# JuanJoZP/cfd-hemodynamic

Measured on NVIDIA B200. Metric: DOF-timesteps/s, higher is better.
Workload: dtype f64

## Files before the change

### cfd_hemodynamic_b200/_lib.py

```python
from __future__ import annotations

import ctypes as C
import os

import numpy as np

_HERE = os.path.dirname(os.path.abspath(__file__))
LIB_PATH = os.path.join(_HERE, "libhemo_sm100.so")

HEMO_DIVERGED = -100
Q_FU, Q_FP, Q_UU, Q_UP, Q_PU, Q_PP = range(6)
CELL_TRIANGLE, CELL_QUADRILATERAL, CELL_TETRAHEDRON, CELL_TRIANGLE_P2 = 0, 1, 2, 3


class HemoError(RuntimeError):
    pass


class HemoDiverged(HemoError):
    pass


class Params(C.Structure):
    _fields_ = [("dt", C.c_double), ("rho", C.c_double), ("mu", C.c_double),
# ... 53 lines not shown
    "hemo_remove_mean_vec": (_I, [_VP, _L, _VP]),
    "hemo_amg_set_level": (_I, [_VP, _I, _I, _I, _I] + [_VP] * 10),
    "hemo_amg_finalize": (_I, [_VP, _I, _I]),
    "hemo_host_aggregate": (_I, [_I, _VP, _VP, _VP, _VP, C.POINTER(_I)]),
    "hemo_set_solver_opts": (_I, [_VP, C.POINTER(SolverOpts)]),
    "hemo_set_pc_mask": (_I, [_VP, _VP]),
    "hemo_set_external_schur": (_I, [_VP, _I]),
    "hemo_amg_setup_scalar": (_I, [_VP, _VP, _D]),
    "hemo_mask_nodes": (_I, [_VP, _VP, _VP]),
    "hemo_vec_mdot": (_I, [_VP, _L, _I, _VP, _L, _VP, _VP]),
    "hemo_vec_maxpy": (_I, [_VP, _L, _I, _VP, _L, _VP, _D, _VP, C.POINTER(_D)]),
    "hemo_vec_scale": (_I, [_VP, _L, _D, _VP, _VP]),
    "hemo_use_graph": (_I, [_VP, _I]),
    "hemo_set_schur_mask": (_I, [_VP, _VP]),
    "hemo_pc_set_schur_operator": (_I, [_VP, _VP, _VP, _VP, _D, _D]),
    "hemo_amg_set_fine_pattern": (_I, [_VP, _I, _VP, _VP]),
    "hemo_pc_set_schur_selfp": (_I, [_VP, _VP, _D]),
    "hemo_pc_set_convection": (_I, [_VP, _VP, _VP, _D]),
    "hemo_pc_setup": (_I, [_VP, _VP, _VP, _VP]),
    "hemo_amg_apply": (_I, [_VP, _I, _VP, _VP, _I]),
    "hemo_amg_get_level_values": (_I, [_VP, _I, _I, _VP, _L]),
    "hemo_pc_apply": (_I, [_VP, _VP, _VP, _VP]),
    "hemo_fgmres": (_I, [_VP, _VP, _VP, _VP, C.POINTER(_I), C.POINTER(_D)]),
    "hemo_comm_unique_id": (_I, [C.c_char_p]),
    "hemo_comm_init": (_I, [_VP, C.c_char_p, _I, _I]),
    "hemo_comm_info": (_I, [_VP, C.POINTER(_I), C.POINTER(_I), C.POINTER(_I), C.POINTER(_L), C.POINTER(_L)]),
    "hemo_comm_set_partition": (_I, [_VP, _I, _I, _VP, _VP, _VP, _VP, _I]),
    "hemo_set_graph": (_I, [_VP, _I, _VP, _VP, _L]),
    "hemo_pc_set_coarse_pressure": (_I, [_VP, _VP, _I] + [_VP] * 6 + [_I]),
    "hemo_comm_halo_update": (_I, [_VP, _VP]),
    "hemo_comm_allreduce": (_I, [_VP, _VP, _I]),
    "hemo_global_dot": (_I, [_VP, _VP, _VP, C.POINTER(_D)]),
    "hemo_set_poll_interval": (_I, [_VP, _I]),
}

_lib = None


def load_library(path: str | None = None):
    global _lib
    if _lib is not None and path is None:
        return _lib
    p = path or LIB_PATH
    if not os.path.exists(p):
        raise HemoError(
            f"{p} not found: build it with `python -m cfd_hemodynamic_b200.build` "
            "(nvcc, sm_100a).  There is no CPU fallback.")
    lib = C.CDLL(p)
    for name, (res, args) in SYMBOLS.items():
        fn = getattr(lib, name)
        fn.restype = res
        fn.argtypes = args
    if path is None:
        _lib = lib
    return lib


def _ptr(t):
    if t is None:
        return None
    return C.c_void_p(t.data_ptr())


def _np_ptr(a: np.ndarray):
    return a.ctypes.data_as(C.c_void_p)

# ... 262 lines not shown
    def amg_set_fine_pattern(self, which, pattern):
        if pattern is None:
            self._check(self.lib.hemo_amg_set_fine_pattern(self._ctx, which, None, None), "hemo_amg_set_fine_pattern")
            return
        rp = np.ascontiguousarray(pattern.indptr, dtype=np.int32)
        ci = np.ascontiguousarray(pattern.indices, dtype=np.int32)
        self._check(self.lib.hemo_amg_set_fine_pattern(self._ctx, which, _np_ptr(rp), _np_ptr(ci)),
                    "hemo_amg_set_fine_pattern")

    def pc_set_schur_selfp(self, vals, coarse_shift=0.0):
        self._check(self.lib.hemo_pc_set_schur_selfp(self._ctx, _ptr(vals), float(coarse_shift)), "hemo_pc_set_schur_selfp")

    def pc_set_convection(self, x, un, coef):
        self._check(self.lib.hemo_pc_set_convection(self._ctx, _ptr(x), _ptr(un), float(coef)), "hemo_pc_set_convection")

    def pc_setup(self, vals, lap=None, mass=None):
        if lap is not None:
            self._keep.update(mass=mass)
        self._check(self.lib.hemo_pc_setup(self._ctx, _ptr(vals), _ptr(lap), _ptr(mass)), "hemo_pc_setup")

    def amg_apply(self, which, b, x, ncycles=1):
        self._check(self.lib.hemo_amg_apply(self._ctx, which, _ptr(b), _ptr(x), ncycles), "hemo_amg_apply")

    def amg_level_values(self, which, level, count):
        t = self.torch
        out = t.empty(count, dtype=t.float64, device=self.device)
        self._check(self.lib.hemo_amg_get_level_values(self._ctx, which, level, _ptr(out), count),
                    "hemo_amg_get_level_values")
        return out

    def pc_apply(self, vals, r, z):
        self._check(self.lib.hemo_pc_apply(self._ctx, _ptr(vals), _ptr(r), _ptr(z)), "hemo_pc_apply")

    @staticmethod
    def comm_unique_id() -> bytes:
        buf = C.create_string_buffer(128)
        rc = load_library().hemo_comm_unique_id(buf)
        if rc:
            raise HemoError("hemo_comm_unique_id failed (NCCL not loadable)")
        return buf.raw

    def comm_init(self, uid: bytes, rank: int, nranks: int):
        self._check(self.lib.hemo_comm_init(self._ctx, C.c_char_p(uid), int(rank), int(nranks)), "hemo_comm_init")

    def comm_info(self):
        r, n, v = C.c_int(), C.c_int(), C.c_int()
        h, a = C.c_int64(), C.c_int64()
        self._check(self.lib.hemo_comm_info(self._ctx, C.byref(r), C.byref(n), C.byref(v), C.byref(h), C.byref(a)),
                    "hemo_comm_info")
        return dict(rank=r.value, nranks=n.value, nccl_version=v.value, halo_updates=h.value, allreduces=a.value)

    def comm_set_partition(self, n_owned, peers, send_ptr, send_nodes, recv_ptr, ras_overlap=False):
        peers = np.ascontiguousarray(peers, dtype=np.int32)
        send_ptr = np.ascontiguousarray(send_ptr, dtype=np.int32)
        send_nodes = np.ascontiguousarray(send_nodes, dtype=np.int32)
        recv_ptr = np.ascontiguousarray(recv_ptr, dtype=np.int32)
        hp = lambda a: a.ctypes.data_as(C.c_void_p)
        self._check(self.lib.hemo_comm_set_partition(self._ctx, int(n_owned), int(peers.shape[0]), hp(peers), hp(send_ptr),
                                                     hp(send_nodes), hp(recv_ptr), int(bool(ras_overlap))),
                    "hemo_comm_set_partition")

    def set_graph(self, rowptr, col):
        self._keep["graph"] = (rowptr, col)
        self.n = int(rowptr.numel() - 1)
        self.nnz_node = int(col.numel())
        self._check(self.lib.hemo_set_graph(self._ctx, self.n, _ptr(rowptr), _ptr(col), self.nnz_node), "hemo_set_graph")
# ... 35 lines not shown
```

### cfd_hemodynamic_b200/csrc/amg.cu

```cuda
#include <cooperative_groups.h>
#include <type_traits>
#include <cub/device/device_scan.cuh>

#include "hemo_internal.cuh"

int hemo_bsr_spmv_ex(hemo_ctx* ctx, int bs, int n, const int32_t* rowptr, const int32_t* col, const areal* val,
                     const areal* x, double alpha, const areal* b, areal* y);

__device__ __forceinline__ int find_col(const int32_t* __restrict__ col, int lo, int hi, int key) {
    int a = lo, b = hi - 1;
    while (a <= b) {
        const int m = (a + b) >> 1;
        const int c = col[m];
        if (c == key) return m;
        if (c < key) a = m + 1; else b = m - 1;
    }
    return -1;
}

template <int BS>
__global__ void __launch_bounds__(256)
k_numeric_ap(int n, const int32_t* __restrict__ a_rowptr, const int32_t* __restrict__ a_col,
             const areal* __restrict__ a_val, const int32_t* __restrict__ p_rowptr,
             const int32_t* __restrict__ p_col, const double* __restrict__ p_val,
// ... 194 lines not shown
                }
        }
#pragma unroll
        for (int k = 0; k < BS; ++k) {
            const double d = (diag[k] != 0.0) ? diag[k] : 1.0;
            dinv[(int64_t)i * BS + k] = 1.0 / d;
            bound = fmax(bound, rs[k] / fabs(d));
        }
    }
    sh[threadIdx.x] = bound;
    __syncthreads();
    for (int s = blockDim.x / 2; s > 0; s >>= 1) {
        if (threadIdx.x < s) sh[threadIdx.x] = fmax(sh[threadIdx.x], sh[threadIdx.x + s]);
        __syncthreads();
    }
    if (threadIdx.x == 0) partial_max[blockIdx.x] = sh[0];
}

__global__ void k_max_final(int m, const double* __restrict__ partial, double* __restrict__ out) {
    __shared__ double sh[256];
    double v = 0.0;
    for (int i = threadIdx.x; i < m; i += blockDim.x) v = fmax(v, partial[i]);
    sh[threadIdx.x] = v;
    __syncthreads();
    for (int s = blockDim.x / 2; s > 0; s >>= 1) {
        if (threadIdx.x < s) sh[threadIdx.x] = fmax(sh[threadIdx.x], sh[threadIdx.x + s]);
        __syncthreads();
    }
    if (threadIdx.x == 0) out[0] = sh[0];
}

__global__ void k_axpy_areal(int64_t n, double a, const areal* __restrict__ x, areal* __restrict__ y) {
    const int64_t i = blockIdx.x * (int64_t)blockDim.x + threadIdx.x;
    if (i < n) y[i] = (areal)fma(a, (double)x[i], (double)y[i]);
}

__global__ void k_to_areal(int64_t n, const double* __restrict__ x, areal* __restrict__ y) {
    const int64_t i = blockIdx.x * (int64_t)blockDim.x + threadIdx.x;
    if (i < n) y[i] = (areal)x[i];
}

__global__ void k_from_areal(int64_t n, const areal* __restrict__ x, double* __restrict__ y) {
    const int64_t i = blockIdx.x * (int64_t)blockDim.x + threadIdx.x;
    if (i < n) y[i] = (double)x[i];
}

template <int BS>
__global__ void k_cheb_start_zero(int64_t N, const areal* __restrict__ dinv, const areal* __restrict__ b,
                                  double inv_theta, areal* __restrict__ r, areal* __restrict__ d,
                                  areal* __restrict__ x) {
    const int64_t i = blockIdx.x * (int64_t)blockDim.x + threadIdx.x;
    if (i >= N) return;
    const double rv = dinv[i] * b[i];
    r[i] = rv;
    const double dv = rv * inv_theta;
    d[i] = dv;
    x[i] = dv;
}

template <int BS>
__device__ __forceinline__ void row_product(const int32_t* __restrict__ rowptr, const int32_t* __restrict__ col,
                                            const areal* __restrict__ val, const areal* __restrict__ x,
                                            int i, bool ok, int lane, double acc[BS]) {
#pragma unroll
    for (int k = 0; k < BS; ++k) acc[k] = 0.0;
    const int r0 = ok ? rowptr[i] : 0, r1 = ok ? rowptr[i + 1] : 0;
    for (int t = r0 + lane; t < r1; t += 12) {
        const int t1 = t + 4, t2 = t + 8;
        const bool p1 = t1 < r1, p2 = t2 < r1;
        const int j0 = col[t];
        const int j1 = p1 ? col[t1] : j0;
        const int j2 = p2 ? col[t2] : j0;
        if (BS == 1) {
            const double v0 = (double)val[t], x0 = (double)x[j0];
            const double v1 = p1 ? (double)val[t1] : 0.0, x1 = (double)x[j1];
            const double v2 = p2 ? (double)val[t2] : 0.0, x2 = (double)x[j2];
            acc[0] = fma(v0, x0, acc[0]);
            acc[0] = fma(v1, x1, acc[0]);
            acc[0] = fma(v2, x2, acc[0]);
        } else {
            const areal2* v2p = reinterpret_cast<const areal2*>(val);
            const areal2* x2p = reinterpret_cast<const areal2*>(x);
            const areal2 a0 = v2p[2 * (int64_t)t], b0 = v2p[2 * (int64_t)t + 1], xa = x2p[j0];
            areal2 a1, b1, a2, b2;
            a1.x = a1.y = b1.x = b1.y = a2.x = a2.y = b2.x = b2.y = 0;
            if (p1) { a1 = v2p[2 * (int64_t)t1]; b1 = v2p[2 * (int64_t)t1 + 1]; }
            if (p2) { a2 = v2p[2 * (int64_t)t2]; b2 = v2p[2 * (int64_t)t2 + 1]; }
            const areal2 xb = x2p[j1], xc = x2p[j2];
            acc[0] += (double)a0.x * xa.x + (double)a0.y * xa.y + (double)a1.x * xb.x + (double)a1.y * xb.y +
                      (double)a2.x * xc.x + (double)a2.y * xc.y;
            acc[BS - 1] += (double)b0.x * xa.x + (double)b0.y * xa.y + (double)b1.x * xb.x + (double)b1.y * xb.y +
                           (double)b2.x * xc.x + (double)b2.y * xc.y;
        }
    }
#pragma unroll
    for (int k = 0; k < BS; ++k) {
        acc[k] += __shfl_xor_sync(0xffffffffu, acc[k], 1, 4);
        acc[k] += __shfl_xor_sync(0xffffffffu, acc[k], 2, 4);
    }
}

template <int BS>
__global__ void __launch_bounds__(256)
k_cheb_start(int n, const int32_t* __restrict__ rowptr, const int32_t* __restrict__ col,
             const areal* __restrict__ val, const areal* __restrict__ dinv, const areal* __restrict__ b,
             double inv_theta, const areal* __restrict__ xin, areal* __restrict__ r, areal* __restrict__ d) {
    const int gt = blockIdx.x * blockDim.x + threadIdx.x;
    const int i = gt >> 2, lane = gt & 3;
    const bool ok = i < n;
    double acc[BS];
    row_product<BS>(rowptr, col, val, xin, i, ok, lane, acc);
    if (ok && lane < BS) {
        const int64_t q = (int64_t)i * BS + lane;
        const double rv = dinv[q] * (b[q] - (lane == 0 ? acc[0] : acc[BS - 1]));
        r[q] = rv;
        d[q] = rv * inv_theta;
    }
}

template <int BS, typename TB>
__global__ void __launch_bounds__(256)
k_presmooth_residual(int n, const int32_t* __restrict__ rowptr, const int32_t* __restrict__ col,
                     const areal* __restrict__ val, const areal* __restrict__ dinv, const TB* __restrict__ b,
                     double inv_theta, areal* __restrict__ x, areal* __restrict__ r, areal* __restrict__ bcopy) {
    const int gt = blockIdx.x * blockDim.x + threadIdx.x;
    const int i = gt >> 2, lane = gt & 3;
    const bool ok = i < n;
    const int r0 = ok ? rowptr[i] : 0, r1 = ok ? rowptr[i + 1] : 0;
    double acc[BS];
#pragma unroll
    for (int k = 0; k < BS; ++k) acc[k] = 0.0;
    for (int t = r0 + lane; t < r1; t += 8) {
        const int t1 = t + 4;
        const bool p1 = t1 < r1;
        const int j0 = col[t];
        const int j1 = p1 ? col[t1] : j0;
        if (BS == 1) {
            const double x0 = (double)dinv[j0] * (double)b[j0] * inv_theta;
            const double x1 = (double)dinv[j1] * (double)b[j1] * inv_theta;
            acc[0] = fma((double)val[t], x0, acc[0]);
            acc[0] = fma(p1 ? (double)val[t1] : 0.0, x1, acc[0]);
        } else {
            const areal2* v2p = reinterpret_cast<const areal2*>(val);
            const areal2 a0 = v2p[2 * (int64_t)t], b0 = v2p[2 * (int64_t)t + 1];
            areal2 a1, b1;
            a1.x = a1.y = b1.x = b1.y = 0;
            if (p1) { a1 = v2p[2 * (int64_t)t1]; b1 = v2p[2 * (int64_t)t1 + 1]; }
            const double xa0 = (double)dinv[2 * (int64_t)j0] * (double)b[2 * (int64_t)j0] * inv_theta;
            const double xa1 = (double)dinv[2 * (int64_t)j0 + 1] * (double)b[2 * (int64_t)j0 + 1] * inv_theta;
            const double xb0 = (double)dinv[2 * (int64_t)j1] * (double)b[2 * (int64_t)j1] * inv_theta;
            const double xb1 = (double)dinv[2 * (int64_t)j1 + 1] * (double)b[2 * (int64_t)j1 + 1] * inv_theta;
            acc[0] += (double)a0.x * xa0 + (double)a0.y * xa1 + (double)a1.x * xb0 + (double)a1.y * xb1;
            acc[BS - 1] += (double)b0.x * xa0 + (double)b0.y * xa1 + (double)b1.x * xb0 + (double)b1.y * xb1;
        }
    }
#pragma unroll
    for (int k = 0; k < BS; ++k) {
        acc[k] += __shfl_xor_sync(0xffffffffu, acc[k], 1, 4);
        acc[k] += __shfl_xor_sync(0xffffffffu, acc[k], 2, 4);
    }
    if (ok && lane < BS) {
        const int64_t q = (int64_t)i * BS + lane;
        const double bv = (double)b[q];
        x[q] = (areal)((double)dinv[q] * bv * inv_theta);
        r[q] = (areal)(bv - (lane == 0 ? acc[0] : acc[BS - 1]));
        if (bcopy) bcopy[q] = (areal)bv;
    }
}

template <int BS>
__global__ void __launch_bounds__(256)
k_cheb_step(int n, const int32_t* __restrict__ rowptr, const int32_t* __restrict__ col,
            const areal* __restrict__ val, const areal* __restrict__ dinv, double c1, double c2,
            const areal* __restrict__ dold, areal* __restrict__ dnew, areal* __restrict__ r,
            areal* __restrict__ x, int add_old, double* __restrict__ x64 ) {
    const int gt = blockIdx.x * blockDim.x + threadIdx.x;
    const int i = gt >> 2, lane = gt & 3;
    const bool ok = i < n;
    double acc[BS];
    row_product<BS>(rowptr, col, val, dold, i, ok, lane, acc);
    if (ok && lane < BS) {
        const int64_t q = (int64_t)i * BS + lane;
        const double rv = r[q] - dinv[q] * (lane == 0 ? acc[0] : acc[BS - 1]);
        r[q] = rv;
        const double dv = c1 * dold[q] + c2 * rv;
        dnew[q] = dv;
        const double xn = (double)x[q] + (add_old ? (dv + (double)dold[q]) : dv);
        x[q] = (areal)xn;
        if (x64) x64[q] = xn;
    }
}

__device__ __forceinline__ int ldg_nc(const int32_t* p) {
    int v;
    asm volatile("ld.global.nc.s32 %0, [%1];" : "=r"(v) : "l"(p));
    return v;
}
__device__ __forceinline__ float ldg_nc(const float* p) {
    float v;
    asm volatile("ld.global.nc.f32 %0, [%1];" : "=f"(v) : "l"(p));
    return v;
}
__device__ __forceinline__ double ldg_nc(const double* p) {
    double v;
    asm volatile("ld.global.nc.f64 %0, [%1];" : "=d"(v) : "l"(p));
    return v;
}
__device__ __forceinline__ float2 ldg_nc(const float2* p) {
    float2 v;
    asm volatile("ld.global.nc.v2.f32 {%0,%1}, [%2];" : "=f"(v.x), "=f"(v.y) : "l"(p));
    return v;
}
__device__ __forceinline__ double2 ldg_nc(const double2* p) {
// ... 15 lines not shown

template <int BS>
struct VecLoad {
    typedef typename std::conditional<BS == 1, areal, areal2>::type raw;
    const areal* __restrict__ x;
    __device__ __forceinline__ raw load(int j) const { return ldg_nc(reinterpret_cast<const raw*>(x) + j); }
    __device__ __forceinline__ void value(const raw& t, double* out) const {
        if constexpr (BS == 1) out[0] = (double)t;
        else { out[0] = (double)t.x; out[1] = (double)t.y; }
    }
};

template <int BS, typename TB>
struct JacobiLoad {
    struct raw { areal d[BS]; TB b[BS]; };
    const areal* __restrict__ dinv;
    const TB* __restrict__ b;
    double inv_theta;
    __device__ __forceinline__ raw load(int j) const {
        raw t;
#pragma unroll
        for (int k = 0; k < BS; ++k) {
            t.d[k] = ldg_nc(dinv + (int64_t)j * BS + k);
            t.b[k] = ldg_nc(b + (int64_t)j * BS + k);
        }
        return t;
    }
    __device__ __forceinline__ void value(const raw& t, double* out) const {
#pragma unroll
        for (int k = 0; k < BS; ++k) out[k] = (double)t.d[k] * (double)t.b[k] * inv_theta;
    }
};

template <int BS, typename XF>
__device__ __forceinline__ void sell_row_product(const int32_t* __restrict__ sptr, const int32_t* __restrict__ scol,
                                                 const areal* __restrict__ sval, int i, const XF xf, double acc[BS]) {
    typedef typename std::conditional<BS == 1, areal, areal4>::type blk;
#pragma unroll
    for (int k = 0; k < BS; ++k) acc[k] = 0.0;
    const int s = i >> 5, lane = i & 31;
    const int base = sptr[s];
    const int W = (sptr[s + 1] - base) >> 5;
    const int32_t* __restrict__ c = scol + base + lane;
    const blk* __restrict__ v = reinterpret_cast<const blk*>(sval) + base + lane;
    for (int k = 0; k < W; k += 4) {
        int kk[4];
        bool ok[4];
#pragma unroll
        for (int u = 0; u < 4; ++u) { ok[u] = k + u < W; kk[u] = 32 * (ok[u] ? k + u : W - 1); }
        int j[4];
        blk a[4];
        typename XF::raw xr[4];
#pragma unroll
        for (int u = 0; u < 4; ++u) j[u] = ldg_nc(c + kk[u]);
#pragma unroll
        for (int u = 0; u < 4; ++u) a[u] = ldg_nc(v + kk[u]);
        __syncwarp();
#pragma unroll
        for (int u = 0; u < 4; ++u) xr[u] = xf.load(j[u]);
        __syncwarp();
#pragma unroll
        for (int u = 0; u < 4; ++u) {
            double xv[BS];
            xf.value(xr[u], xv);
            if constexpr (BS == 1) {
                acc[0] = fma(ok[u] ? (double)a[u] : 0.0, xv[0], acc[0]);
            } else {
                const double m = ok[u] ? 1.0 : 0.0;
                acc[0] += m * ((double)a[u].x * xv[0] + (double)a[u].y * xv[1]);
                acc[1] += m * ((double)a[u].z * xv[0] + (double)a[u].w * xv[1]);
            }
        }
    }
}

template <int BS>
__global__ void __launch_bounds__(256)
k_sell_cheb_start(int n, const int32_t* __restrict__ sptr, const int32_t* __restrict__ scol, const areal* __restrict__ sval,
                  const areal* __restrict__ dinv, const areal* __restrict__ b, double inv_theta,
                  const areal* __restrict__ xin, areal* __restrict__ r, areal* __restrict__ d) {
    const int i = blockIdx.x * blockDim.x + threadIdx.x;
    if (i >= n) return;
    double acc[BS];
    sell_row_product<BS>(sptr, scol, sval, i, VecLoad<BS>{xin}, acc);
#pragma unroll
    for (int k = 0; k < BS; ++k) {
        const int64_t q = (int64_t)i * BS + k;
        const double rv = (double)dinv[q] * ((double)b[q] - acc[k]);
        r[q] = (areal)rv;
        d[q] = (areal)(rv * inv_theta);
    }
}

template <int BS, typename TB>
__global__ void __launch_bounds__(256)
k_sell_presmooth_residual(int n, const int32_t* __restrict__ sptr, const int32_t* __restrict__ scol,
                          const areal* __restrict__ sval, const areal* __restrict__ dinv, const TB* __restrict__ b,
                          double inv_theta, areal* __restrict__ x, areal* __restrict__ r, areal* __restrict__ bcopy) {
    const int i = blockIdx.x * blockDim.x + threadIdx.x;
    if (i >= n) return;
    double acc[BS];
    sell_row_product<BS>(sptr, scol, sval, i, JacobiLoad<BS, TB>{dinv, b, inv_theta}, acc);
#pragma unroll
    for (int k = 0; k < BS; ++k) {
        const int64_t q = (int64_t)i * BS + k;
        const double bv = (double)b[q];
        x[q] = (areal)((double)dinv[q] * bv * inv_theta);
        r[q] = (areal)(bv - acc[k]);
        if (bcopy) bcopy[q] = (areal)bv;
    }
}

template <int BS>
__global__ void __launch_bounds__(256)
k_sell_cheb_step(int n, const int32_t* __restrict__ sptr, const int32_t* __restrict__ scol, const areal* __restrict__ sval,
                 const areal* __restrict__ dinv, double c1, double c2, const areal* __restrict__ dold,
                 areal* __restrict__ dnew, areal* __restrict__ r, areal* __restrict__ x, int add_old,
                 double* __restrict__ x64) {
    const int i = blockIdx.x * blockDim.x + threadIdx.x;
    if (i >= n) return;
    double acc[BS];
    sell_row_product<BS>(sptr, scol, sval, i, VecLoad<BS>{dold}, acc);
#pragma unroll
    for (int k = 0; k < BS; ++k) {
        const int64_t q = (int64_t)i * BS + k;
        const double dq = (double)dold[q];
        const double rv = (double)r[q] - (double)dinv[q] * acc[k];
        r[q] = (areal)rv;
        const double dv = c1 * dq + c2 * rv;
        dnew[q] = (areal)dv;
        const double xn = (double)x[q] + (add_old ? (dv + dq) : dv);
        x[q] = (areal)xn;
        if (x64) x64[q] = xn;
    }
}

template <int BS>
__global__ void __launch_bounds__(256)
k_sell_residual(int n, const int32_t* __restrict__ sptr, const int32_t* __restrict__ scol, const areal* __restrict__ sval,
                const areal* __restrict__ x, const areal* __restrict__ b, areal* __restrict__ y) {
    const int i = blockIdx.x * blockDim.x + threadIdx.x;
    if (i >= n) return;
    double acc[BS];
    sell_row_product<BS>(sptr, scol, sval, i, VecLoad<BS>{x}, acc);
#pragma unroll
    for (int k = 0; k < BS; ++k) {
        const int64_t q = (int64_t)i * BS + k;
        y[q] = (areal)((double)b[q] - acc[k]);
    }
}

__global__ void k_sell_fill_col(int n, int nrows_padded, const int32_t* __restrict__ rowptr, const int32_t* __restrict__ col,
                                const int32_t* __restrict__ sptr, int32_t* __restrict__ scol) {
    const int i = blockIdx.x * blockDim.x + threadIdx.x;
    if (i >= nrows_padded) return;
    const int s = i >> 5, lane = i & 31;
    const int base = sptr[s], W = (sptr[s + 1] - base) >> 5;
    const int r0 = i < n ? rowptr[i] : 0, deg = i < n ? rowptr[i + 1] - r0 : 0;
    const int self = i < n ? i : n - 1;
    for (int k = 0; k < W; ++k) scol[base + 32 * k + lane] = k < deg ? col[r0 + k] : self;
}

template <int BS>
__global__ void __launch_bounds__(256)
k_sell_fill_val(int n, const int32_t* __restrict__ rowptr, const areal* __restrict__ val,
                const int32_t* __restrict__ sptr, areal* __restrict__ sval) {
    const int gt = blockIdx.x * blockDim.x + threadIdx.x;
    const int i = gt >> 2, sub = gt & 3;
    if (i >= n) return;
    const int base = sptr[i >> 5] + (i & 31);
    const int r0 = rowptr[i], deg = rowptr[i + 1] - r0;
    for (int k = sub; k < deg; k += 4) {
#pragma unroll
        for (int c = 0; c < BS * BS; ++c)
            sval[((int64_t)base + 32 * k) * (BS * BS) + c] = val[((int64_t)r0 + k) * (BS * BS) + c];
    }
}

template <int BS>
__global__ void __launch_bounds__(256)
k_prolong_add_row(int nrows, const int32_t* __restrict__ rowptr, const int32_t* __restrict__ col,
                  const double* __restrict__ w, const areal* __restrict__ x, areal* __restrict__ y) {
    const int i = blockIdx.x * blockDim.x + threadIdx.x;
    if (i >= nrows) return;
    const int r0 = rowptr[i], r1 = rowptr[i + 1];
    double acc[BS];
#pragma unroll
    for (int k = 0; k < BS; ++k) acc[k] = 0.0;
    for (int t = r0; t < r1; ++t) {
        const int j = col[t];
        const double wt = w[t];
#pragma unroll
        for (int k = 0; k < BS; ++k) acc[k] = fma(wt, (double)x[(int64_t)j * BS + k], acc[k]);
    }
#pragma unroll
    for (int k = 0; k < BS; ++k) {
        const int64_t q = (int64_t)i * BS + k;
        y[q] = (areal)((double)y[q] + acc[k]);
    }
}

template <int BS, bool ADD>
__global__ void __launch_bounds__(256)
k_transfer(int nrows, const int32_t* __restrict__ rowptr, const int32_t* __restrict__ col,
           const double* __restrict__ w, const areal* __restrict__ x, areal* __restrict__ y) {
    const int gt = blockIdx.x * blockDim.x + threadIdx.x;
    const int I = gt >> 2, lane = gt & 3;
    const bool ok = I < nrows;
    const int r0 = ok ? rowptr[I] : 0, r1 = ok ? rowptr[I + 1] : 0;
    double acc[BS];
#pragma unroll
    for (int k = 0; k < BS; ++k) acc[k] = 0.0;
    for (int t = r0 + lane; t < r1; t += 12) {
        const int t1 = t + 4, t2 = t + 8;
        const bool p1 = t1 < r1, p2 = t2 < r1;
        const int j0 = col[t];
        const int j1 = p1 ? col[t1] : j0;
        const int j2 = p2 ? col[t2] : j0;
        const double w0 = w[t], w1 = p1 ? w[t1] : 0.0, w2 = p2 ? w[t2] : 0.0;
#pragma unroll
        for (int k = 0; k < BS; ++k) {
            const double x0 = (double)x[(int64_t)j0 * BS + k], x1 = (double)x[(int64_t)j1 * BS + k],
                         x2 = (double)x[(int64_t)j2 * BS + k];
            acc[k] += w0 * x0 + w1 * x1 + w2 * x2;
        }
    }
#pragma unroll
    for (int k = 0; k < BS; ++k) {
        acc[k] += __shfl_xor_sync(0xffffffffu, acc[k], 1, 4);
        acc[k] += __shfl_xor_sync(0xffffffffu, acc[k], 2, 4);
    }
    if (ok && lane < BS) {
        const double v = (lane == 0) ? acc[0] : acc[BS - 1];
        const int64_t q = (int64_t)I * BS + lane;
        if (ADD) y[q] = (areal)((double)y[q] + v);
        else y[q] = (areal)v;
    }
}

namespace cg = cooperative_groups;

struct CtaScope {
    __device__ __forceinline__ int tid() const { return threadIdx.x; }
    __device__ __forceinline__ int nthreads() const { return blockDim.x; }
    __device__ __forceinline__ void sync() const { __syncthreads(); }
};
struct GridScope {
    cg::grid_group g;
    __device__ __forceinline__ GridScope() : g(cg::this_grid()) {}
    __device__ __forceinline__ int tid() const { return blockIdx.x * blockDim.x + threadIdx.x; }
    __device__ __forceinline__ int nthreads() const { return gridDim.x * blockDim.x; }
    __device__ __forceinline__ void sync() const { g.sync(); }
// ... 157 lines not shown
        areal* x = (nl == 1) ? x0 : desc[nl - 1].x;
        const int lane = tid & 7, group = tid >> 3, ngroups = T >> 3;
        for (int base = 0; base < dense_n; base += ngroups) {
            const int row = base + group;
            const bool ok = row < dense_n;
            double acc = 0.0;
            if (ok)
                for (int c = lane; c < dense_n; c += 8) acc = fma(dense_inv[(int64_t)row * dense_n + c], (double)b[c], acc);
            acc += __shfl_xor_sync(0xffffffffu, acc, 1, 8);
            acc += __shfl_xor_sync(0xffffffffu, acc, 2, 8);
            acc += __shfl_xor_sync(0xffffffffu, acc, 4, 8);
            if (ok && lane == 0) x[row] = (areal)acc;
        }
        sc.sync();
    }
    for (int l = nl - 2; l >= 0; --l) {
        const HemoCoarseLevel L = desc[l];
        const areal* b = (l == 0) ? b0 : L.b;
        areal* x = (l == 0) ? x0 : L.x;
        const areal* xc = desc[l + 1].x;
        rows_transfer<BS>(sc, L.n, L.p_rowptr, L.p_col, L.p_val, xc, [&](int i, const double* acc) {
#pragma unroll
            for (int k = 0; k < BS; ++k) x[i * BS + k] = (areal)((double)x[i * BS + k] + acc[k]);
        });
        sc.sync();
        fused_smooth<BS>(sc, L, b, x, false, degree, ratio);
    }
}

template <int BS>
__global__ void __launch_bounds__(1024)
k_coarse_vcycle(const HemoCoarseLevel* __restrict__ desc, int nl, const areal* __restrict__ b0, areal* __restrict__ x0,
                int degree_pre, int degree, double ratio, const double* __restrict__ dense_inv, int dense_n) {
    CtaScope sc;
    coarse_vcycle_body<BS>(sc, desc, nl, b0, x0, degree_pre, degree, ratio, dense_inv, dense_n);
}

template <int BS>
__global__ void __launch_bounds__(1024)
k_coarse_vcycle_cluster(const HemoCoarseLevel* __restrict__ desc, int nl, const areal* __restrict__ b0, areal* __restrict__ x0,
                        int degree_pre, int degree, double ratio, const double* __restrict__ dense_inv, int dense_n) {
    ClusterScope sc;
    coarse_vcycle_body<BS>(sc, desc, nl, b0, x0, degree_pre, degree, ratio, dense_inv, dense_n);
}

template <int BS>
__global__ void __launch_bounds__(512)
k_coarse_vcycle_grid(const HemoCoarseLevel* __restrict__ desc, int nl, const areal* __restrict__ b0, areal* __restrict__ x0,
                     int degree_pre, int degree, double ratio, const double* __restrict__ dense_inv, int dense_n) {
    GridScope sc;
    coarse_vcycle_body<BS>(sc, desc, nl, b0, x0, degree_pre, degree, ratio, dense_inv, dense_n);
}

template <int BS>
__global__ void k_dense_fill(int n, const int32_t* __restrict__ rowptr, const int32_t* __restrict__ col,
                             const areal* __restrict__ val, int N, double shift_rel, double* __restrict__ M ) {
    const int i = blockIdx.x * blockDim.x + threadIdx.x;
    if (i >= n) return;
    for (int t = rowptr[i]; t < rowptr[i + 1]; ++t) {
        const int j = col[t];
#pragma unroll
        for (int k = 0; k < BS; ++k)
#pragma unroll
            for (int l = 0; l < BS; ++l) {
                double v = val[(int64_t)t * BS * BS + k * BS + l];
                if (i == j && k == l) v *= (1.0 + shift_rel);
// ... 11 lines not shown
    const int total = N * N;
    for (int q = tid; q < total; q += blockDim.x) A[q] = Min[q];
    __syncthreads();
    for (int p = 0; p < N; ++p) {
        if (tid == 0) {
            const double piv = A[p * N + p];
            if (!(fabs(piv) > 0.0) || !isfinite(piv)) *fail = 1;
            pivinv = 1.0 / piv;
            A[p * N + p] = 1.0;
        }
        __syncthreads();
        const double pi = pivinv;
        for (int c = tid; c < N; c += blockDim.x) A[p * N + c] *= pi;
        for (int r = tid; r < N; r += blockDim.x) {
            if (r != p) { fcol[r] = A[r * N + p]; A[r * N + p] = 0.0; }
            else fcol[r] = 0.0;
        }
        __syncthreads();
        for (int q = tid; q < total; q += blockDim.x) {
            const int r = q / N;
            const int c = q - r * N;
            const double f = fcol[r];
            if (f != 0.0) A[q] -= f * A[p * N + c];
        }
        __syncthreads();
    }
    for (int q = tid; q < total; q += blockDim.x) inv[q] = A[q];
}

__global__ void __launch_bounds__(256)
k_dense_gemv(int N, const double* __restrict__ inv, const areal* __restrict__ b, areal* __restrict__ y) {
    const int row = (blockIdx.x * blockDim.x + threadIdx.x) >> 5;
    const int lane = threadIdx.x & 31;
    double acc = 0.0;
    if (row < N)
        for (int c = lane; c < N; c += 32) acc += inv[(int64_t)row * N + c] * b[c];
#pragma unroll
    for (int o = 16; o > 0; o >>= 1) acc += __shfl_down_sync(0xffffffffu, acc, o);
    if (row < N && lane == 0) y[row] = acc;
}

static void free_level(HemoAmgLevel& L) {
    cudaFree(L.p_rowptr); cudaFree(L.p_col); cudaFree(L.p_val);
    cudaFree(L.r_rowptr); cudaFree(L.r_col); cudaFree(L.r_val);
    cudaFree(L.ap_rowptr); cudaFree(L.ap_col); cudaFree(L.ap_val);
    cudaFree(L.c_rowptr); cudaFree(L.c_col);
    cudaFree(L.ap_seg_ptr); cudaFree(L.ap_seg_src); cudaFree(L.c_seg_ptr); cudaFree(L.c_seg_src);
    L = HemoAmgLevel();
}

void hemo_amg_free(HemoAmg* amg) {
    for (int l = 0; l < HEMO_MAX_LEVELS; ++l) {
        free_level(amg->lev[l]);
        HemoAmgOp& o = amg->op[l];
        cudaFree(o.val); cudaFree(o.dinv); cudaFree(o.x); cudaFree(o.b); cudaFree(o.r); cudaFree(o.d);
        cudaFree(o.sell_ptr); cudaFree(o.sell_col); cudaFree(o.sell_val);
        o = HemoAmgOp();
    }
    if (amg->apply_exec) { cudaGraphExecDestroy(amg->apply_exec); amg->apply_exec = nullptr; }
    amg->apply_valid = false;
    cudaFree(amg->fine_rowptr); cudaFree(amg->fine_col); cudaFree(amg->fine_rowof);
    amg->fine_rowptr = amg->fine_col = amg->fine_rowof = nullptr; amg->fine_nnz = 0;
    cudaFree(amg->dense_inv); cudaFree(amg->dense_work); cudaFree(amg->fuse_desc); cudaFree(amg->lmax_dev);
    amg->fuse_desc = nullptr; amg->lmax_dev = nullptr; amg->fuse_level = amg->fuse_level_grid = amg->fuse_level_cluster = amg->fuse_base = -1;
    amg->grid_blocks = amg->cluster_ctas = 0;
    amg->dense_inv = amg->dense_work = nullptr;
// ... 289 lines not shown
        HEMO_CHECK_CUDA(ctx, cudaMemcpyAsync(&fail_h, fail, sizeof(int), cudaMemcpyDeviceToHost, st));
        HEMO_CHECK_CUDA(ctx, cudaStreamSynchronize(st));
        if (fail_h) HEMO_FAIL(ctx, HEMO_DIVERGED, "coarsest AMG operator is singular");
    }
    for (int l = 0; l + 1 < amg->nlev; ++l) {
        double b = ctx->red_host[64 + l];
        if (!(b > 0.0) || !isfinite(b)) HEMO_FAIL(ctx, HEMO_DIVERGED, "AMG operator has a non-finite Gershgorin bound");
        amg->op[l].lmax = b;
    }
    return 0;
}

int hemo_amg_numeric_shift(hemo_ctx* ctx, HemoAmg* amg, double coarse_shift) {
    if (!amg->ready) HEMO_FAIL(ctx, HEMO_ESTATE, "AMG hierarchy not finalized");
    amg->apply_valid = false;
    if (amg->bs == 2) return amg_numeric_t<2>(ctx, amg, coarse_shift);
    return amg_numeric_t<1>(ctx, amg, coarse_shift);
}

int hemo_amg_numeric(hemo_ctx* ctx, HemoAmg* amg) { return hemo_amg_numeric_shift(ctx, amg, 0.0); }

template <int BS>
static int smooth_t(hemo_ctx* ctx, const HemoAmgOp& A, const areal* b, areal* x, bool x_is_zero, int degree,
                    double ratio, double* x64 = nullptr, bool* wrote64 = nullptr) {
    cudaStream_t st = ctx->stream;
    const double lmax = A.lmax, lmin = lmax / ratio;
    const double theta = 0.5 * (lmax + lmin), delta = 0.5 * (lmax - lmin);
    const double sigma = theta / delta;
    double rho = 1.0 / sigma;
    const int64_t N = (int64_t)A.n * BS;
    areal* d0 = A.d;
    areal* d1 = A.d + N;
    if (x_is_zero) {
        k_cheb_start_zero<BS><<<hemo_grid(N, 256), 256, 0, st>>>(N, A.dinv, b, 1.0 / theta, A.r, d0, x);
    } else if (A.sell_ptr) {
        k_sell_cheb_start<BS><<<hemo_grid(A.n, 256), 256, 0, st>>>(A.n, A.sell_ptr, A.sell_col, A.sell_val, A.dinv, b, 1.0 / theta,
                                                                    x, A.r, d0);
    } else {
        k_cheb_start<BS><<<hemo_grid((int64_t)A.n * 4, 256), 256, 0, st>>>(A.n, A.rowptr, A.col, A.val, A.dinv, b, 1.0 / theta, x,
                                                              A.r, d0);
    }
    HEMO_LAUNCH_CHECK(ctx);
    bool pending = !x_is_zero;
    for (int k = 1; k < degree; ++k) {
        const double rho_new = 1.0 / (2.0 * sigma - rho);
        const double c1 = rho_new * rho, c2 = 2.0 * rho_new / delta;
        const bool fine = (A.n == ctx->n);
        if (fine) HEMO_PROF_BEGIN(ctx, BS == 2 ? HEMO_PROF_CHEB_U0 : HEMO_PROF_CHEB_P0);
        const bool last = (k == degree - 1);
        if (A.sell_ptr)
            k_sell_cheb_step<BS><<<hemo_grid(A.n, 256), 256, 0, st>>>(A.n, A.sell_ptr, A.sell_col, A.sell_val, A.dinv, c1, c2, d0, d1,
                                                                       A.r, x, pending ? 1 : 0, last ? x64 : nullptr);
        else
            k_cheb_step<BS><<<hemo_grid((int64_t)A.n * 4, 256), 256, 0, st>>>(A.n, A.rowptr, A.col, A.val, A.dinv, c1, c2, d0, d1, A.r, x,
                                                                 pending ? 1 : 0, last ? x64 : nullptr);
        if (last && x64 && wrote64) *wrote64 = true;
        HEMO_LAUNCH_CHECK(ctx);
        if (fine) HEMO_PROF_END(ctx, BS == 2 ? HEMO_PROF_CHEB_U0 : HEMO_PROF_CHEB_P0);
        pending = false;
        areal* t = d0; d0 = d1; d1 = t;
        rho = rho_new;
    }
    if (pending) {
        k_axpy_areal<<<hemo_grid(N, 256), 256, 0, st>>>(N, 1.0, d0, x);
        HEMO_LAUNCH_CHECK(ctx);
    }
    return 0;
}

template <int BS>
static int vcycle_t(hemo_ctx* ctx, HemoAmg* amg, int l, const areal* b, areal* x, bool x_is_zero,
                    const double* b64 = nullptr, double* x64 = nullptr, bool* wrote64 = nullptr) {
    cudaStream_t st = ctx->stream;
    const HemoAmgOp& A = amg->op[l];
    const int degree = ctx->opts.cheb_degree > 0 ? ctx->opts.cheb_degree : 2;
    const int degree_pre = ctx->opts.cheb_degree_pre > 0 ? ctx->opts.cheb_degree_pre : degree;
    const double ratio = ctx->opts.cheb_ratio > 1.0 ? ctx->opts.cheb_ratio : 4.0;
    if (l == amg->fuse_level_grid && amg->grid_blocks > 0) {
        const HemoCoarseLevel* desc = amg->fuse_desc + (l - amg->fuse_base);
        int nl = amg->nlev - l, dp = degree_pre, dg = degree, dn = amg->dense_n;
        double rt = ratio;
        const double* dinv = amg->dense_inv;
        void* args[] = {(void*)&desc, (void*)&nl, (void*)&b, (void*)&x, (void*)&dp, (void*)&dg, (void*)&rt, (void*)&dinv, (void*)&dn};
        const void* fn = (BS == 2) ? (const void*)k_coarse_vcycle_grid<2> : (const void*)k_coarse_vcycle_grid<1>;
        cudaError_t e = cudaLaunchCooperativeKernel(fn, dim3(amg->grid_blocks), dim3(512), args, 0, st);
        if (e == cudaSuccess) {
            ctx->launches++;
            return 0;
        }
        cudaGetLastError();
        ctx->amg[0].grid_blocks = ctx->amg[1].grid_blocks = 0;
        if (ctx->capturing) HEMO_FAIL(ctx, HEMO_ERETRY, "cooperative launch not capturable: capture is repeated without it");
    }
    if (l == amg->fuse_level_cluster && amg->cluster_ctas > 0) {
        cudaLaunchConfig_t cfg = {};
        cfg.gridDim = dim3(amg->cluster_ctas); cfg.blockDim = dim3(1024); cfg.stream = st;
        cudaLaunchAttribute at[1];
        at[0].id = cudaLaunchAttributeClusterDimension;
        at[0].val.clusterDim.x = amg->cluster_ctas; at[0].val.clusterDim.y = 1; at[0].val.clusterDim.z = 1;
        cfg.attrs = at; cfg.numAttrs = 1;
        const HemoCoarseLevel* desc = amg->fuse_desc + (l - amg->fuse_base);
        const double* dinv = amg->dense_inv;
        HEMO_CHECK_CUDA(ctx, cudaLaunchKernelEx(&cfg, k_coarse_vcycle_cluster<BS>, desc, amg->nlev - l, b, x, degree_pre, degree,
                                                ratio, dinv, amg->dense_n));
        ctx->launches++;
        return 0;
    }
    if (l == amg->fuse_level) {
        k_coarse_vcycle<BS><<<1, 1024, 0, st>>>(amg->fuse_desc + (l - amg->fuse_base), amg->nlev - l, b, x, degree_pre, degree, ratio,
                                                amg->dense_inv, amg->dense_n);
        HEMO_LAUNCH_CHECK(ctx);
        return 0;
    }
    if (l == amg->nlev - 1) {
        const int N = amg->dense_n;
        k_dense_gemv<<<hemo_grid((int64_t)N * 32, 256), 256, 0, st>>>(N, amg->dense_inv, b, x);
        HEMO_LAUNCH_CHECK(ctx);
        return 0;
    }
    int rc;
    if (x_is_zero && degree_pre == 1) {
        const double lmax = A.lmax, lmin = lmax / ratio;
        const double inv_theta = 1.0 / (0.5 * (lmax + lmin));
        const int g = hemo_grid((int64_t)A.n * 4, 256);
        if (A.sell_ptr) {
            const int gs = hemo_grid(A.n, 256);
            if (b64) k_sell_presmooth_residual<BS, double><<<gs, 256, 0, st>>>(A.n, A.sell_ptr, A.sell_col, A.sell_val, A.dinv, b64,
                                                                                inv_theta, x, A.r, const_cast<areal*>(b));
            else k_sell_presmooth_residual<BS, areal><<<gs, 256, 0, st>>>(A.n, A.sell_ptr, A.sell_col, A.sell_val, A.dinv, b,
                                                                          inv_theta, x, A.r, nullptr);
        } else if (b64) k_presmooth_residual<BS, double><<<g, 256, 0, st>>>(A.n, A.rowptr, A.col, A.val, A.dinv, b64, inv_theta, x, A.r,
                                                                      const_cast<areal*>(b));
        else k_presmooth_residual<BS, areal><<<g, 256, 0, st>>>(A.n, A.rowptr, A.col, A.val, A.dinv, b, inv_theta, x, A.r, nullptr);
        HEMO_LAUNCH_CHECK(ctx);
    } else {
        if (b64) {
            const int64_t N = (int64_t)A.n * BS;
            k_to_areal<<<hemo_grid(N, 256), 256, 0, st>>>(N, b64, const_cast<areal*>(b));
            HEMO_LAUNCH_CHECK(ctx);
        }
        if ((rc = smooth_t<BS>(ctx, A, b, x, x_is_zero, degree_pre, ratio))) return rc;
        if (A.sell_ptr) {
            k_sell_residual<BS><<<hemo_grid(A.n, 256), 256, 0, st>>>(A.n, A.sell_ptr, A.sell_col, A.sell_val, x, b, A.r);
            HEMO_LAUNCH_CHECK(ctx);
        } else if ((rc = hemo_bsr_spmv_ex(ctx, BS, A.n, A.rowptr, A.col, A.val, x, -1.0, b, A.r))) return rc;
    }
    const HemoAmgLevel& L = amg->lev[l];
    HemoAmgOp& C = amg->op[l + 1];
    k_transfer<BS, false><<<hemo_grid((int64_t)C.n * 4, 256), 256, 0, st>>>(C.n, L.r_rowptr, L.r_col, L.r_val, A.r, C.b);
    HEMO_LAUNCH_CHECK(ctx);
    if ((rc = vcycle_t<BS>(ctx, amg, l + 1, C.b, C.x, true))) return rc;
    if (L.nnz_p <= 6 * (int64_t)A.n && A.n >= 32768)
        k_prolong_add_row<BS><<<hemo_grid(A.n, 256), 256, 0, st>>>(A.n, L.p_rowptr, L.p_col, L.p_val, C.x, x);
    else
        k_transfer<BS, true><<<hemo_grid((int64_t)A.n * 4, 256), 256, 0, st>>>(A.n, L.p_rowptr, L.p_col, L.p_val, C.x, x);
    HEMO_LAUNCH_CHECK(ctx);
    if ((rc = smooth_t<BS>(ctx, A, b, x, false, degree, ratio, x64, wrote64))) return rc;
    return 0;
}

int hemo_amg_vcycle(hemo_ctx* ctx, HemoAmg* amg, const double* b, double* x, int ncycles) {
    if (!amg->ready) HEMO_FAIL(ctx, HEMO_ESTATE, "AMG hierarchy not finalized");
    int rc;
    HemoAmgOp& top = amg->op[0];
    const int64_t N = (int64_t)top.n * amg->bs;
    const int nc = ncycles > 0 ? ncycles : 1;
    const bool per_level_top = amg->nlev > 1 && amg->fuse_level != 0 && !(amg->fuse_level_grid == 0 && amg->grid_blocks > 0);
    if (!per_level_top) {
        k_to_areal<<<hemo_grid(N, 256), 256, 0, ctx->stream>>>(N, b, top.b);
        HEMO_LAUNCH_CHECK(ctx);
    }
    bool wrote64 = false;
    for (int c = 0; c < nc; ++c) {
        const double* b64 = (per_level_top && c == 0) ? b : nullptr;
        double* x64 = (per_level_top && c == nc - 1) ? x : nullptr;
        if (amg->bs == 2) rc = vcycle_t<2>(ctx, amg, 0, top.b, top.x, c == 0, b64, x64, &wrote64);
        else rc = vcycle_t<1>(ctx, amg, 0, top.b, top.x, c == 0, b64, x64, &wrote64);
        if (rc) return rc;
    }
    if (!wrote64) {
        k_from_areal<<<hemo_grid(N, 256), 256, 0, ctx->stream>>>(N, top.x, x);
        HEMO_LAUNCH_CHECK(ctx);
    }
    return 0;
}
```

### cfd_hemodynamic_b200/csrc/comm.cu

```cuda
#include <dlfcn.h>
#include <string.h>

#include "hemo_internal.cuh"

typedef struct ncclComm* ncclComm_t;
typedef struct { char internal[128]; } ncclUniqueId;
typedef int ncclResult_t;
enum { ncclFloat64 = 8, ncclSum = 0 };

struct NcclApi {
    void* lib = nullptr;
    ncclResult_t (*GetUniqueId)(ncclUniqueId*) = nullptr;
    ncclResult_t (*CommInitRank)(ncclComm_t*, int, ncclUniqueId, int) = nullptr;
    ncclResult_t (*CommDestroy)(ncclComm_t) = nullptr;
    ncclResult_t (*AllReduce)(const void*, void*, size_t, int, int, ncclComm_t, cudaStream_t) = nullptr;
    ncclResult_t (*Send)(const void*, size_t, int, int, ncclComm_t, cudaStream_t) = nullptr;
    ncclResult_t (*Recv)(void*, size_t, int, int, ncclComm_t, cudaStream_t) = nullptr;
    ncclResult_t (*GroupStart)() = nullptr;
    ncclResult_t (*GroupEnd)() = nullptr;
    const char* (*GetErrorString)(ncclResult_t) = nullptr;
    ncclResult_t (*GetVersion)(int*) = nullptr;
};

static NcclApi g_nccl;
// ... 46 lines not shown
        ncclResult_t _r = (expr);                                                      \
        if (_r != 0) {                                                                 \
            (ctx)->err = std::string(#expr) + ": " + g_nccl.GetErrorString(_r);        \
            return 1000 + (int)_r;                                                     \
        }                                                                              \
    } while (0)

extern "C" int hemo_comm_unique_id(char* out128) {
    if (!out128) return HEMO_EINVAL;
    if (nccl_load()) return HEMO_ESTATE;
    ncclUniqueId id;
    if (g_nccl.GetUniqueId(&id) != 0) return HEMO_ESTATE;
    memcpy(out128, id.internal, 128);
    return 0;
}

extern "C" int hemo_comm_init(hemo_ctx* ctx, const char* uid128, int rank, int nranks) {
    if (!ctx || !uid128 || nranks < 1 || rank < 0 || rank >= nranks) return HEMO_EINVAL;
    const char* e = nccl_load();
    if (e) HEMO_FAIL(ctx, HEMO_ESTATE, e);
    hemo_comm_free(ctx);
    HemoComm* c = new HemoComm();
    c->rank = rank; c->nranks = nranks;
    ncclUniqueId id;
    memcpy(id.internal, uid128, 128);
    HEMO_CHECK_CUDA(ctx, cudaSetDevice(ctx->device));
    ncclResult_t r = g_nccl.CommInitRank(&c->comm, nranks, id, rank);
    if (r != 0) {
        ctx->err = std::string("ncclCommInitRank: ") + g_nccl.GetErrorString(r);
        delete c;
        return 1000 + (int)r;
    }
    ctx->comm = c;
    return 0;
}

extern "C" int hemo_comm_info(hemo_ctx* ctx, int* rank, int* nranks, int* nccl_version, int64_t* halo_updates,
                              int64_t* allreduces) {
    if (!ctx || !ctx->comm) return HEMO_ESTATE;
    if (rank) *rank = ctx->comm->rank;
    if (nranks) *nranks = ctx->comm->nranks;
    if (nccl_version) g_nccl.GetVersion(nccl_version);
    if (halo_updates) *halo_updates = ctx->comm->halo_updates;
    if (allreduces) *allreduces = ctx->comm->allreduces;
    return 0;
}

void hemo_comm_free(hemo_ctx* ctx) {
    HemoComm* c = ctx->comm;
    if (!c) return;
    cudaStreamSynchronize(ctx->stream);
    cudaFree(c->send_nodes); cudaFree(c->sendbuf);
    if (c->comm && g_nccl.CommDestroy) g_nccl.CommDestroy(c->comm);
    delete c;
    ctx->comm = nullptr;
}

extern "C" int hemo_comm_set_partition(hemo_ctx* ctx, int n_owned, int nneigh, const int32_t* peers_host,
                                       const int32_t* send_ptr_host, const int32_t* send_nodes_host,
                                       const int32_t* recv_ptr_host, int ras_overlap) {
    if (!ctx || n_owned < 0 || nneigh < 0 || nneigh > HEMO_MAX_NEIGH) return HEMO_EINVAL;
    if (!ctx->comm) HEMO_FAIL(ctx, HEMO_ESTATE, "hemo_comm_init must precede hemo_comm_set_partition");
    if (!ctx->cells) HEMO_FAIL(ctx, HEMO_ESTATE, "hemo_set_mesh must precede hemo_comm_set_partition");
    if (n_owned > ctx->n) return HEMO_EINVAL;
    if (nneigh && (!peers_host || !send_ptr_host || !send_nodes_host || !recv_ptr_host)) return HEMO_EINVAL;
    HemoComm* c = ctx->comm;
// ... 90 lines not shown
```

### cfd_hemodynamic_b200/csrc/hemo_internal.cuh

```cuda
#pragma once
#include <cuda_runtime.h>
#include <stdint.h>
#include <stdio.h>
#include <string>
#include <vector>

#include "../../include/hemo.h"
#include "hemo_rules.h"

#define HEMO_MAXQ 80
#define HEMO_NRULES 6
#define HEMO_MAX_FACET_SETS 8
#define HEMO_MAX_LEVELS 16
#define HEMO_DENSE_MAX 160

#ifdef HEMO_AMG_FP64
typedef double areal;
typedef double2 areal2;
typedef double4 areal4;
#else
typedef float areal;
typedef float2 areal2;
typedef float4 areal4;
#endif
// ... 84 lines not shown
};

enum { HEMO_PROF_SPMV = 0, HEMO_PROF_CELL_JAC = 1, HEMO_PROF_GATHER_MAT = 2, HEMO_PROF_CELL_RES = 3,
       HEMO_PROF_CHEB_U0 = 4, HEMO_PROF_CHEB_P0 = 5, HEMO_PROF_MDOT = 6, HEMO_PROF_MAXPY = 7,
       HEMO_PROF_RAP = 8, HEMO_PROF_HALO = 9, HEMO_PROF_ALLREDUCE = 10, HEMO_PROF_COARSE = 11, HEMO_PROF_PC = 12,
       HEMO_PROF_NCLASS = 13 };

struct HemoProf {
    bool on = false;
    std::vector<cudaEvent_t> ev[HEMO_PROF_NCLASS];
    size_t used[HEMO_PROF_NCLASS] = {0};
};

struct hemo_tet_state;
struct hemo_cc_state;
struct HemoComm;

struct HemoKrylov {
    int m = 0;
    int64_t ldv = 0;
    double* H = nullptr;
    double* small = nullptr;
    double* partial = nullptr;
    double* state = nullptr;
    double* state_host = nullptr;
    int last_its = 0;
    int poll_every = 1;
    int64_t polls = 0;
    int64_t seg_len0 = 0, seg_off1 = 0, seg_len1 = 0;
    cudaGraphExec_t iter_exec = nullptr;
    bool iter_valid = false;
    const double* iter_vals = nullptr;
    int64_t iter_nodes = 0;
};

struct hemo_ctx {
    HemoProf prof;
    hemo_tet_state* tet = nullptr;
    hemo_cc_state* cc = nullptr;
    int formulation = 0;
    int64_t rule_version = 0;
    int device = 0;
    cudaStream_t stream = 0;
    std::string err;
    int64_t launches = 0;

    int nv = 3;
    int dim = 2;
    double fz = 0.0;
    const double* x = nullptr;
    const int32_t* cells = nullptr;
    const double* h = nullptr;
    int n = 0, E = 0;
    const int32_t* nrowptr = nullptr;
    const int32_t* ncol = nullptr;
    int64_t nnz_node = 0;
    int32_t* cellpos = nullptr;
    int32_t* mseg_ptr = nullptr;
    int32_t* mseg_src = nullptr;
    int32_t* vseg_ptr = nullptr;
    int32_t* vseg_src = nullptr;
    int32_t* diagslot = nullptr;
    int32_t* rowof = nullptr;
    double* Ae = nullptr;
    double* Fe = nullptr;
    size_t Ae_count = 0, Fe_count = 0;
    int external_schur = 0;
    double* dvec = nullptr;

    HemoForm par{0, 0, 0, {0, 0}, 0, 0.5, 1.0, 0, 0, 0, 0};
    bool have_par = false;
    const double* uh = nullptr;
    HemoRule rules[HEMO_NRULES];
    bool have_rule[HEMO_NRULES] = {false, false, false, false, false, false};
    bool rules_dirty = true;
    HemoQuadRule* qrules = nullptr;
    bool qrules_dirty = true;
    void* p2rules = nullptr;
// ... 51 lines not shown
    HemoComm* comm = nullptr;
    int comm_ras_overlap = 0;
};

#define HEMO_CHECK_CUDA(ctx, expr)                                                     \
    do {                                                                               \
        cudaError_t _e = (expr);                                                       \
        if (_e != cudaSuccess) {                                                       \
            (ctx)->err = std::string(#expr) + ": " + cudaGetErrorString(_e);           \
            return (int)_e;                                                            \
        }                                                                              \
    } while (0)

#define HEMO_FAIL(ctx, code, msg)  \
    do {                           \
        (ctx)->err = (msg);        \
        return (code);             \
    } while (0)

#define HEMO_2D_ONLY(ctx, what)                                                                      \
    do {                                                                                             \
        if ((ctx)->dim == 3) HEMO_FAIL(ctx, HEMO_ESTATE, what " is not implemented for tetrahedra yet"); \
    } while (0)

#define HEMO_LAUNCH_CHECK(ctx)                                       \
    do {                                                             \
        (ctx)->launches++;                                           \
        cudaError_t _e = cudaGetLastError();                         \
        if (_e != cudaSuccess) {                                     \
            (ctx)->err = std::string("kernel launch: ") +            \
                         cudaGetErrorString(_e) + " at " + __FILE__ + ":" + std::to_string(__LINE__); \
            return (int)_e;                                          \
        }                                                            \
    } while (0)

static inline void hemo_prof_mark(hemo_ctx* ctx, int cls) {
    if (!ctx->prof.on || ctx->capturing) return;
    HemoProf& p = ctx->prof;
    if (p.used[cls] == p.ev[cls].size()) {
        cudaEvent_t e;
        cudaEventCreate(&e);
        p.ev[cls].push_back(e);
    }
    cudaEventRecord(p.ev[cls][p.used[cls]++], ctx->stream);
}
#define HEMO_PROF_BEGIN(ctx, cls) hemo_prof_mark(ctx, cls)
#define HEMO_PROF_END(ctx, cls) hemo_prof_mark(ctx, cls)

template <typename T>
static inline int hemo_alloc(hemo_ctx* ctx, T** p, size_t count) {
    if (*p) { cudaFree(*p); *p = nullptr; }
    if (count == 0) return 0;
    HEMO_CHECK_CUDA(ctx, cudaMalloc((void**)p, count * sizeof(T)));
    return 0;
}

template <typename T>
static inline int hemo_upload(hemo_ctx* ctx, T** p, const T* src, size_t count, bool src_is_device) {
    int rc = hemo_alloc(ctx, p, count);
    if (rc) return rc;
    if (count == 0) return 0;
    HEMO_CHECK_CUDA(ctx, cudaMemcpyAsync(*p, src, count * sizeof(T),
                                         src_is_device ? cudaMemcpyDeviceToDevice : cudaMemcpyHostToDevice,
                                         ctx->stream));
    return 0;
}
// ... 48 lines not shown
```

### cfd_hemodynamic_b200/csrc/krylov.cu

```cuda
#include <math.h>

#include "hemo_internal.cuh"

#define FG_BLOCKS 1184
#define FG_THREADS 256
#define FG_TILE 8

int hemo_remove_mean(hemo_ctx* ctx, int64_t n, double* x);
int hemo_pc_apply_body(hemo_ctx* ctx, const double* vals_dev, const double* r_dev, double* z_dev);

struct FgState {
    int j;
    int its;
    int converged;
    int cycle_full;
    double res, tol, bnorm, beta;
    unsigned int ticket_mdot, ticket_maxpy, ticket_misc, pad;
};

struct FgSeg {
    int64_t len0, off1, len1;
};
__device__ __forceinline__ int64_t seg_index(const FgSeg& s, int64_t i) { return i < s.len0 ? i : i - s.len0 + s.off1; }
__device__ __forceinline__ bool seg_owned(const FgSeg& s, int64_t q) { return q < s.len0 || (q >= s.off1 && q < s.off1 + s.len1); }
// ... 50 lines not shown
    s = fg_block_sum(s, sh);
    if (threadIdx.x == 0) out[0] = s;
}

__global__ void k_fg_begin_cycle(FgState* st, const double* __restrict__ normsq, int first, double rtol, double atol,
                                 double* __restrict__ g, double* __restrict__ scale, int m) {
    if (threadIdx.x != 0 || blockIdx.x != 0) return;
    if (!first && st->converged) return;
    const double beta = sqrt(fmax(normsq[0], 0.0));
    if (first) {
        st->its = 0;
        st->converged = 0;
        st->bnorm = beta;
        st->tol = fmax(rtol * beta, atol);
        st->res = beta;
        if (beta == 0.0 || beta <= atol) st->converged = 1;
        else if (!isfinite(beta)) st->converged = -1;
    } else {
        st->res = beta;
        if (beta <= st->tol) st->converged = 1;
        else if (!isfinite(beta)) st->converged = -1;
    }
    st->beta = beta;
    st->j = 0;
    st->cycle_full = 0;
    for (int i = 0; i <= m; ++i) g[i] = 0.0;
    g[0] = beta;
    scale[0] = beta > 0.0 ? 1.0 / beta : 0.0;
}

__global__ void __launch_bounds__(FG_THREADS)
k_fg_load(const FgState* __restrict__ st, int64_t n, const double* __restrict__ V, int64_t ldv,
          const double* __restrict__ scale, double* __restrict__ pc_in) {
    if (st->converged || st->cycle_full) return;
    const int j = st->j;
    const double s = scale[j];
    const double* v = V + (int64_t)j * ldv;
    for (int64_t i = blockIdx.x * (int64_t)blockDim.x + threadIdx.x; i < n; i += (int64_t)gridDim.x * blockDim.x)
        pc_in[i] = s * v[i];
}

__global__ void __launch_bounds__(256)
k_fg_spmv_node(const FgState* __restrict__ st, int n, int64_t nnz_node, const int32_t* __restrict__ nrowptr,
               const int32_t* __restrict__ ncol, const double* __restrict__ vals, const double* __restrict__ z,
               double* __restrict__ V, double* __restrict__ Z, int64_t ldv) {
    if (st->converged || st->cycle_full) return;
    const int j = st->j;
    const double* xu = z;
    const double* xp = z + 2 * (int64_t)n;
    double* w = V + (int64_t)(j + 1) * ldv;
    double* zj = Z + (int64_t)j * ldv;
    const int gt = blockIdx.x * blockDim.x + threadIdx.x;
    const int i = gt >> 3;
    const int lane = gt & 7;
    const bool ok = i < n;
    const int r0 = ok ? nrowptr[i] : 0;
    const int deg = ok ? nrowptr[i + 1] - r0 : 0;
    const int64_t ru0 = 6 * (int64_t)r0, ru1 = ru0 + 3 * deg, rp = 6 * nnz_node + 3 * (int64_t)r0;
    double a0 = 0.0, a1 = 0.0, a2 = 0.0;
    for (int t = lane; t < deg; t += 8) {
        const int c = ncol[r0 + t];
        const double2 xv = reinterpret_cast<const double2*>(xu)[c];
        const double x2 = xp[c];
        a0 += vals[ru0 + 2 * t] * xv.x + vals[ru0 + 2 * t + 1] * xv.y + vals[ru0 + 2 * deg + t] * x2;
        a1 += vals[ru1 + 2 * t] * xv.x + vals[ru1 + 2 * t + 1] * xv.y + vals[ru1 + 2 * deg + t] * x2;
        a2 += vals[rp + 2 * t] * xv.x + vals[rp + 2 * t + 1] * xv.y + vals[rp + 2 * deg + t] * x2;
    }
#pragma unroll
    for (int o = 4; o > 0; o >>= 1) {
        a0 += __shfl_down_sync(0xffffffffu, a0, o, 8);
        a1 += __shfl_down_sync(0xffffffffu, a1, o, 8);
        a2 += __shfl_down_sync(0xffffffffu, a2, o, 8);
    }
    if (ok && lane == 0) {
        reinterpret_cast<double2*>(w)[i] = make_double2(a0, a1);
        w[2 * (int64_t)n + i] = a2;
        reinterpret_cast<double2*>(zj)[i] = reinterpret_cast<const double2*>(xu)[i];
        zj[2 * (int64_t)n + i] = xp[i];
    }
}

__global__ void __launch_bounds__(FG_THREADS)
k_fg_store(const FgState* __restrict__ st, int64_t n, const double* __restrict__ z, const double* __restrict__ w,
           double* __restrict__ V, double* __restrict__ Z, int64_t ldv) {
    if (st->converged || st->cycle_full) return;
    const int j = st->j;
    double* wj = V + (int64_t)(j + 1) * ldv;
    double* zj = Z + (int64_t)j * ldv;
    for (int64_t i = blockIdx.x * (int64_t)blockDim.x + threadIdx.x; i < n; i += (int64_t)gridDim.x * blockDim.x) {
        zj[i] = z[i];
        wj[i] = w[i];
    }
}

template <bool SEG>
__global__ void __launch_bounds__(FG_THREADS)
k_fg_mdot(const FgState* __restrict__ st, FgSeg seg, const double* __restrict__ V, int64_t ldv,
          double* __restrict__ partial , int kpad) {
    extern __shared__ double acc_sh[];
    if (st->converged || st->cycle_full) return;
    const int j = st->j, k = j + 1;
    const double* w = V + (int64_t)k * ldv;
    const int64_t n = seg.len0 + seg.len1;
    const int64_t tile = (int64_t)FG_THREADS * FG_TILE;
    const int64_t ntiles = (n + tile - 1) / tile;
    const int lane = threadIdx.x & 31, wid = threadIdx.x >> 5, nw = FG_THREADS / 32;
    for (int i = threadIdx.x; i < nw * kpad; i += blockDim.x) acc_sh[i] = 0.0;
    __syncthreads();
    double* acc = acc_sh + wid * kpad;
    for (int64_t tl = blockIdx.x; tl < ntiles; tl += gridDim.x) {
        const int64_t base = tl * tile + threadIdx.x;
        double wr[FG_TILE];
        int64_t qi[FG_TILE];
#pragma unroll
        for (int e = 0; e < FG_TILE; ++e) {
            const int64_t idx = base + (int64_t)e * FG_THREADS;
            const bool ok = idx < n;
            qi[e] = ok ? (SEG ? seg_index(seg, idx) : idx) : 0;
            wr[e] = ok ? w[qi[e]] : 0.0;
        }
        for (int i = 0; i < k; i += 4) {
            const double* V0 = V + (int64_t)i * ldv;
            const double* V1 = V + (int64_t)min(i + 1, k - 1) * ldv;
            const double* V2 = V + (int64_t)min(i + 2, k - 1) * ldv;
            const double* V3 = V + (int64_t)min(i + 3, k - 1) * ldv;
            double a0 = 0.0, a1 = 0.0, a2 = 0.0, a3 = 0.0;
#pragma unroll
            for (int e = 0; e < FG_TILE; ++e) {
                a0 = fma(V0[qi[e]], wr[e], a0);
                a1 = fma(V1[qi[e]], wr[e], a1);
                a2 = fma(V2[qi[e]], wr[e], a2);
                a3 = fma(V3[qi[e]], wr[e], a3);
            }
#pragma unroll
            for (int o = 16; o > 0; o >>= 1) {
                a0 += __shfl_down_sync(0xffffffffu, a0, o);
                a1 += __shfl_down_sync(0xffffffffu, a1, o);
                a2 += __shfl_down_sync(0xffffffffu, a2, o);
                a3 += __shfl_down_sync(0xffffffffu, a3, o);
            }
            if (lane == 0) {
                acc[i] += a0;
                if (i + 1 < k) acc[i + 1] += a1;
                if (i + 2 < k) acc[i + 2] += a2;
                if (i + 3 < k) acc[i + 3] += a3;
            }
        }
    }
    __syncthreads();
    for (int i = threadIdx.x; i < k; i += blockDim.x) {
        double s = 0.0;
#pragma unroll
        for (int q = 0; q < nw; ++q) s += acc_sh[q * kpad + i];
        partial[(int64_t)i * gridDim.x + blockIdx.x] = s;
    }
}

__global__ void __launch_bounds__(128)
k_fg_mdot_final(const FgState* __restrict__ st, int nblk, const double* __restrict__ partial,
                const double* __restrict__ scale, double* __restrict__ hcol) {
    __shared__ double sh[32];
    if (st->converged || st->cycle_full) return;
    const int i = blockIdx.x;
    if (i > st->j) return;
    double s = 0.0;
    for (int b = threadIdx.x; b < nblk; b += blockDim.x) s += partial[(int64_t)i * nblk + b];
    s = fg_block_sum(s, sh);
    if (threadIdx.x == 0) hcol[i] = scale[i] * s;
}

__device__ void fg_givens(FgState* st, int m, const double* __restrict__ hcol, double hn, double* __restrict__ H,
                          double* __restrict__ cs, double* __restrict__ sn, double* __restrict__ g,
                          double* __restrict__ scale, double* __restrict__ smem ) {
    const int j = st->j;
    double* hs = smem;
    double* cs_s = smem + (m + 2);
    double* sn_s = smem + 2 * (m + 2);
    for (int i = threadIdx.x; i <= j; i += blockDim.x) {
        hs[i] = hcol[i];
        if (i < j) { cs_s[i] = cs[i]; sn_s[i] = sn[i]; }
    }
    __syncthreads();
    if (threadIdx.x == 0) {
        hs[j + 1] = hn;
        for (int i = 0; i < j; ++i) {
            const double a = hs[i], b = hs[i + 1];
            hs[i] = cs_s[i] * a + sn_s[i] * b;
            hs[i + 1] = -sn_s[i] * a + cs_s[i] * b;
        }
        const double a = hs[j], b = hs[j + 1];
        const double d = hypot(a, b);
        const double c = d > 0.0 ? a / d : 1.0, sgn = d > 0.0 ? b / d : 0.0;
        cs[j] = c;
        sn[j] = sgn;
        hs[j] = d;
        hs[j + 1] = 0.0;
        const double gj = g[j];
        g[j + 1] = -sgn * gj;
        g[j] = c * gj;
        const double res = fabs(sgn * gj);
        st->res = res;
        st->its += 1;
        scale[j + 1] = hn > 0.0 ? 1.0 / hn : 0.0;
        if (!isfinite(res)) st->converged = -1;
        else if (res <= st->tol) st->converged = 1;
        else if (hn == 0.0) st->converged = 2;
        if (j + 1 >= m) st->cycle_full = 1;
    }
    __syncthreads();
    double* Hj = H + (int64_t)j * (m + 1);
    for (int i = threadIdx.x; i <= j + 1; i += blockDim.x) Hj[i] = hs[i];
    __syncthreads();
    if (threadIdx.x == 0) st->j = j + 1;
}

__global__ void __launch_bounds__(FG_THREADS)
k_fg_maxpy(FgState* st, FgSeg seg, int64_t nloc, double* __restrict__ V, int64_t ldv, const double* __restrict__ hcol, int m,
           double* __restrict__ partial, double* __restrict__ normsq_out, int do_givens, double* __restrict__ H,
           double* __restrict__ cs, double* __restrict__ sn, double* __restrict__ g, double* __restrict__ scale) {
    __shared__ double sh[32];
    extern __shared__ double hsh[];
    if (st->converged || st->cycle_full) return;
    const int j = st->j, k = j + 1;
    double* w = V + (int64_t)k * ldv;
    for (int i = threadIdx.x; i < k; i += blockDim.x) hsh[i] = hcol[i] * scale[i];
    __syncthreads();
    double nrm = 0.0;
    for (int64_t q = blockIdx.x * (int64_t)blockDim.x + threadIdx.x; q < nloc; q += (int64_t)gridDim.x * blockDim.x) {
        double acc = w[q];
        for (int i = 0; i < k; ++i) acc = fma(-hsh[i], V[(int64_t)i * ldv + q], acc);
        w[q] = acc;
        if (seg_owned(seg, q)) nrm = fma(acc, acc, nrm);
    }
    nrm = fg_block_sum(nrm, sh);
    if (threadIdx.x == 0) partial[blockIdx.x] = nrm;
    if (!fg_last_block(&st->ticket_maxpy)) return;
    __shared__ double total;
    double s = 0.0;
    for (int b = threadIdx.x; b < (int)gridDim.x; b += blockDim.x) s += partial[b];
    s = fg_block_sum(s, sh);
    if (threadIdx.x == 0) {
        normsq_out[0] = s;
        total = s;
    }
    __syncthreads();
    if (do_givens) fg_givens(st, m, hcol, sqrt(fmax(total, 0.0)), H, cs, sn, g, scale, hsh);
}

__global__ void k_fg_givens(FgState* st, int m, const double* __restrict__ hcol, const double* __restrict__ normsq,
                            double* __restrict__ H, double* __restrict__ cs, double* __restrict__ sn,
                            double* __restrict__ g, double* __restrict__ scale) {
    extern __shared__ double gsh[];
    if (st->converged || st->cycle_full) return;
    fg_givens(st, m, hcol, sqrt(fmax(normsq[0], 0.0)), H, cs, sn, g, scale, gsh);
}

__global__ void k_fg_backsolve(FgState* st, int m, const double* __restrict__ H, const double* __restrict__ g,
                               double* __restrict__ ycoef, int* __restrict__ kout) {
    if (threadIdx.x != 0 || blockIdx.x != 0) return;
    const int k = st->j;
    for (int i = k - 1; i >= 0; --i) {
        double s = g[i];
        for (int l = i + 1; l < k; ++l) s -= H[(int64_t)l * (m + 1) + i] * ycoef[l];
        ycoef[i] = s / H[(int64_t)i * (m + 1) + i];
    }
    *kout = k;
}

__global__ void __launch_bounds__(FG_THREADS)
k_fg_update(const int* __restrict__ kptr, int64_t n, const double* __restrict__ Z, int64_t ldv,
            const double* __restrict__ ycoef, double* __restrict__ y) {
    extern __shared__ double csh[];
    const int k = *kptr;
    for (int i = threadIdx.x; i < k; i += blockDim.x) csh[i] = ycoef[i];
    __syncthreads();
    for (int64_t idx = blockIdx.x * (int64_t)blockDim.x + threadIdx.x; idx < n; idx += (int64_t)gridDim.x * blockDim.x) {
        double acc = y[idx];
        for (int i = 0; i < k; ++i) acc = fma(csh[i], Z[(int64_t)i * ldv + idx], acc);
        y[idx] = acc;
    }
}

__global__ void __launch_bounds__(FG_THREADS)
k_fg_residual(const FgState* __restrict__ st, int64_t n, const double* __restrict__ b, const double* __restrict__ Ay,
              double* __restrict__ r) {
// ... 47 lines not shown
}

struct FgPtrs {
    FgState* st;
    double *H, *cs, *sn, *g, *ycoef, *hcol, *scale, *normsq;
    int* kout;
};

static FgPtrs fg_ptrs(hemo_ctx* ctx) {
    HemoKrylov& K = ctx->kry;
    const int m = K.m;
    FgPtrs p;
    p.st = reinterpret_cast<FgState*>(K.state);
    p.normsq = K.state + 16;
    p.kout = reinterpret_cast<int*>(K.state + 24);
    p.H = K.H;
    p.cs = K.small;
    p.sn = K.small + (m + 2);
    p.g = K.small + 2 * (m + 2);
    p.ycoef = K.small + 3 * (m + 2);
    p.hcol = K.small + 4 * (m + 2);
    p.scale = K.small + 5 * (m + 2);
    return p;
}

static int fg_iteration_body(hemo_ctx* ctx, const double* vals_dev) {
    HemoKrylov& K = ctx->kry;
    const FgPtrs p = fg_ptrs(ctx);
    const int n = ctx->n, m = K.m;
    const int64_t N = (int64_t)(ctx->dim + 1) * n, ldv = K.ldv;
    cudaStream_t st = ctx->stream;
    const FgSeg seg = {K.seg_len0 ? K.seg_len0 : N, K.seg_off1, K.seg_len0 ? K.seg_len1 : 0};
    int rc;
    k_fg_load<<<fg_grid(N, 4), FG_THREADS, 0, st>>>(p.st, N, ctx->kry_V, ldv, p.scale, ctx->pc_in);
    HEMO_LAUNCH_CHECK(ctx);
    if (ctx->comm && ctx->comm_ras_overlap && (rc = hemo_comm_halo(ctx, ctx->pc_in))) return rc;
    HEMO_PROF_BEGIN(ctx, HEMO_PROF_PC);
    if ((rc = hemo_pc_apply_body(ctx, vals_dev, ctx->pc_in, ctx->pc_out))) return rc;
    HEMO_PROF_END(ctx, HEMO_PROF_PC);
    if (ctx->comm && (rc = hemo_comm_halo(ctx, ctx->pc_out))) return rc;
    HEMO_PROF_BEGIN(ctx, HEMO_PROF_SPMV);
    if (ctx->dim == 3) {
        if ((rc = hemo_tet_spmv(ctx, vals_dev, ctx->pc_out, ctx->kry_w))) return rc;
        k_fg_store<<<fg_grid(N, 4), FG_THREADS, 0, st>>>(p.st, N, ctx->pc_out, ctx->kry_w, ctx->kry_V, ctx->kry_Z, ldv);
    } else {
        k_fg_spmv_node<<<hemo_grid((int64_t)n * 8, 256), 256, 0, st>>>(p.st, n, ctx->nnz_node, ctx->nrowptr, ctx->ncol, vals_dev,
                                                                    ctx->pc_out, ctx->kry_V, ctx->kry_Z, ldv);
    }
    HEMO_LAUNCH_CHECK(ctx);
    HEMO_PROF_END(ctx, HEMO_PROF_SPMV);
    const int64_t nown = seg.len0 + seg.len1;
    HEMO_PROF_BEGIN(ctx, HEMO_PROF_MDOT);
    {
        const int kpad = m + 4;
        const int gm = fg_grid(nown, FG_TILE);
        const size_t smem = sizeof(double) * (FG_THREADS / 32) * kpad;
        if (seg.len1 > 0) k_fg_mdot<true><<<gm, FG_THREADS, smem, st>>>(p.st, seg, ctx->kry_V, ldv, K.partial, kpad);
        else k_fg_mdot<false><<<gm, FG_THREADS, smem, st>>>(p.st, seg, ctx->kry_V, ldv, K.partial, kpad);
        HEMO_LAUNCH_CHECK(ctx);
        k_fg_mdot_final<<<m, 128, 0, st>>>(p.st, gm, K.partial, p.scale, p.hcol);
        HEMO_LAUNCH_CHECK(ctx);
    }
    HEMO_PROF_END(ctx, HEMO_PROF_MDOT);
    if (ctx->comm && (rc = hemo_comm_allreduce_j(ctx, p.hcol, m + 1))) return rc;
    HEMO_PROF_BEGIN(ctx, HEMO_PROF_MAXPY);
    k_fg_maxpy<<<fg_grid(N, 1), FG_THREADS, sizeof(double) * 3 * (m + 2), st>>>(p.st, seg, N, ctx->kry_V, ldv, p.hcol, m, K.partial,
                                                                               p.normsq, ctx->comm ? 0 : 1, p.H, p.cs, p.sn, p.g,
                                                                               p.scale);
    HEMO_LAUNCH_CHECK(ctx);
    HEMO_PROF_END(ctx, HEMO_PROF_MAXPY);
    if (ctx->comm) {
        if ((rc = hemo_comm_allreduce_j(ctx, p.normsq, 1))) return rc;
        k_fg_givens<<<1, 64, sizeof(double) * 3 * (m + 2), st>>>(p.st, m, p.hcol, p.normsq, p.H, p.cs, p.sn, p.g, p.scale);
        HEMO_LAUNCH_CHECK(ctx);
    }
    return 0;
}

static int fg_iteration(hemo_ctx* ctx, const double* vals_dev) {
    HemoKrylov& K = ctx->kry;
    const bool graph_ok = ctx->use_graph && ctx->stream != 0 && !ctx->prof.on;
    if (!graph_ok) return fg_iteration_body(ctx, vals_dev);
    if (K.iter_valid && K.iter_exec && K.iter_vals == vals_dev) {
        HEMO_CHECK_CUDA(ctx, cudaGraphLaunch(K.iter_exec, ctx->stream));
        ctx->launches += K.iter_nodes;
        return 0;
    }
    cudaStream_t st = ctx->stream;
    const int64_t before = ctx->launches;
    ctx->capturing = true;
    if (cudaStreamBeginCapture(st, cudaStreamCaptureModeThreadLocal) != cudaSuccess) {
        ctx->capturing = false;
        cudaGetLastError();
        return fg_iteration_body(ctx, vals_dev);
    }
    int rc = fg_iteration_body(ctx, vals_dev);
    cudaGraph_t g = nullptr;
    cudaError_t e = cudaStreamEndCapture(st, &g);
    ctx->capturing = false;
    K.iter_nodes = ctx->launches - before;
    ctx->launches = before;
    if (rc != 0 || e != cudaSuccess || !g) {
        cudaGetLastError();
        if (g) cudaGraphDestroy(g);
        if (rc == HEMO_ERETRY) return fg_iteration(ctx, vals_dev);
        if (rc) return rc;
        ctx->use_graph = 0;
        return fg_iteration_body(ctx, vals_dev);
    }
    bool updated = false;
    if (K.iter_exec) {
        cudaGraphExecUpdateResultInfo info;
        if (cudaGraphExecUpdate(K.iter_exec, g, &info) == cudaSuccess) updated = true;
        else { cudaGetLastError(); cudaGraphExecDestroy(K.iter_exec); K.iter_exec = nullptr; }
    }
    if (!updated) {
        e = cudaGraphInstantiate(&K.iter_exec, g, 0);
        if (e != cudaSuccess) { cudaGraphDestroy(g); HEMO_CHECK_CUDA(ctx, e); }
    }
    cudaGraphDestroy(g);
    K.iter_valid = true;
    K.iter_vals = vals_dev;
    HEMO_CHECK_CUDA(ctx, cudaGraphLaunch(K.iter_exec, st));
    ctx->launches += K.iter_nodes;
    return 0;
}

static int fg_poll(hemo_ctx* ctx, FgState* out) {
    HemoKrylov& K = ctx->kry;
    HEMO_CHECK_CUDA(ctx, cudaMemcpyAsync(K.state_host, K.state, sizeof(FgState), cudaMemcpyDeviceToHost, ctx->stream));
    HEMO_CHECK_CUDA(ctx, cudaStreamSynchronize(ctx->stream));
    *out = *reinterpret_cast<FgState*>(K.state_host);
    K.polls++;
    return 0;
}

extern "C" int hemo_set_poll_interval(hemo_ctx* ctx, int every) {
    if (!ctx || every < 1) return HEMO_EINVAL;
    ctx->kry.poll_every = every;
    return 0;
}

extern "C" int hemo_fgmres(hemo_ctx* ctx, const double* vals_dev, const double* b_dev, double* y_dev, int* its_out,
                           double* rel_resid_out) {
    if (!ctx || !vals_dev || !b_dev || !y_dev) return HEMO_EINVAL;
    if (!ctx->mass || !ctx->pc_tmp_u) HEMO_FAIL(ctx, HEMO_ESTATE, "hemo_pc_setup not called");
    const int n = ctx->n;
    const int64_t N = (int64_t)(ctx->dim + 1) * n;
    const int64_t ldv = (N + 31) / 32 * 32;
    const int m = ctx->opts.restart;
    cudaStream_t st = ctx->stream;
    int rc;
    if ((rc = fg_ensure(ctx, m, ldv))) return rc;
    HemoKrylov& K = ctx->kry;
    const FgPtrs p = fg_ptrs(ctx);
    const FgSeg seg = {K.seg_len0 ? K.seg_len0 : N, K.seg_off1, K.seg_len0 ? K.seg_len1 : 0};
    const int64_t nown = seg.len0 + seg.len1;
// ... 50 lines not shown
```

### cfd_hemodynamic_b200/csrc/linalg.cu

```cuda
#include "hemo_internal.cuh"

#define RED_BLOCKS 1184
#define RED_THREADS 256

static void drop_graphs(hemo_ctx* ctx) {
    hemo_krylov_invalidate(ctx);
    if (ctx->pc_graph_exec) { cudaGraphExecDestroy(ctx->pc_graph_exec); ctx->pc_graph_exec = nullptr; }
    if (ctx->pc_graph) { cudaGraphDestroy(ctx->pc_graph); ctx->pc_graph = nullptr; }
    ctx->pc_graph_dirty = true;
    for (int w = 0; w < 2; ++w) {
        HemoAmg& a = ctx->amg[w];
        if (a.apply_exec) { cudaGraphExecDestroy(a.apply_exec); a.apply_exec = nullptr; }
        a.apply_valid = false;
    }
}

int hemo_ensure_reduce(hemo_ctx* ctx, size_t partial_n, size_t out_n) {
    const size_t min_partial = (size_t)RED_BLOCKS * 404, min_out = 1024;
    if (partial_n < min_partial) partial_n = min_partial;
    if (out_n < min_out) out_n = min_out;
    if (partial_n > ctx->red_partial_n) {
        if (ctx->red_partial) {
            HEMO_CHECK_CUDA(ctx, cudaStreamSynchronize(ctx->stream));
            drop_graphs(ctx);
// ... 120 lines not shown
    cudaStream_t st = ctx->stream;
#define LAUNCH(RU, RP, CU, CP)                                                                        \
    k_spmv_node<RU, RP, CU, CP><<<grid, 256, 0, st>>>(n, ctx->nnz_node, ctx->nrowptr, ctx->ncol, vals, \
                                                      xu, xp, alpha, bu, bp, yu, yp)
    if (rows == 3 && cols == 3) LAUNCH(true, true, true, true);
    else if (rows == 1 && cols == 1) LAUNCH(true, false, true, false);
    else if (rows == 1 && cols == 2) LAUNCH(true, false, false, true);
    else if (rows == 2 && cols == 1) LAUNCH(false, true, true, false);
    else if (rows == 2 && cols == 2) LAUNCH(false, true, false, true);
    else HEMO_FAIL(ctx, HEMO_EINVAL, "unsupported sub-block");
#undef LAUNCH
    HEMO_LAUNCH_CHECK(ctx);
    return 0;
}

extern "C" int hemo_spmv(hemo_ctx* ctx, const double* vals_dev, const double* x_dev, double* y_dev) {
    if (!ctx || !vals_dev || !x_dev || !y_dev) return HEMO_EINVAL;
    if (!ctx->nrowptr) HEMO_FAIL(ctx, HEMO_ESTATE, "node graph not set");
    if (ctx->dim == 3) return hemo_tet_spmv(ctx, vals_dev, x_dev, y_dev);
    const int64_t n = ctx->n;
    return hemo_spmv_block(ctx, 3, 3, vals_dev, x_dev, x_dev + 2 * n, 1.0, nullptr, nullptr, y_dev, y_dev + 2 * n);
}

template <int BS>
__global__ void __launch_bounds__(256)
k_bsr_spmv(int n, const int32_t* __restrict__ rowptr, const int32_t* __restrict__ col,
           const areal* __restrict__ val, const areal* __restrict__ x, double alpha,
           const areal* __restrict__ b, areal* __restrict__ y) {
    const int gt = blockIdx.x * blockDim.x + threadIdx.x;
    const int i = gt >> 2;
    const int lane = gt & 3;
    const bool ok = i < n;
    const int r0 = ok ? rowptr[i] : 0, r1 = ok ? rowptr[i + 1] : 0;
    double a0 = 0.0, a1 = 0.0;
    for (int t = r0 + lane; t < r1; t += 12) {
        const int t1 = t + 4, t2 = t + 8;
        const bool p1 = t1 < r1, p2 = t2 < r1;
        const int j0 = col[t];
        const int j1 = p1 ? col[t1] : j0;
        const int j2 = p2 ? col[t2] : j0;
        if (BS == 1) {
            const double v0 = (double)val[t], x0 = (double)x[j0];
            const double v1 = p1 ? (double)val[t1] : 0.0, x1 = (double)x[j1];
            const double v2 = p2 ? (double)val[t2] : 0.0, x2 = (double)x[j2];
            a0 = fma(v0, x0, a0);
            a0 = fma(v1, x1, a0);
            a0 = fma(v2, x2, a0);
        } else {
            const areal2* v2p = reinterpret_cast<const areal2*>(val);
            const areal2* x2p = reinterpret_cast<const areal2*>(x);
            const areal2 c0 = v2p[2 * (int64_t)t], d0 = v2p[2 * (int64_t)t + 1], xa = x2p[j0];
            areal2 c1, d1, c2, d2;
            c1.x = c1.y = d1.x = d1.y = c2.x = c2.y = d2.x = d2.y = 0;
            if (p1) { c1 = v2p[2 * (int64_t)t1]; d1 = v2p[2 * (int64_t)t1 + 1]; }
            if (p2) { c2 = v2p[2 * (int64_t)t2]; d2 = v2p[2 * (int64_t)t2 + 1]; }
            const areal2 xb = x2p[j1], xc = x2p[j2];
            a0 += (double)c0.x * xa.x + (double)c0.y * xa.y + (double)c1.x * xb.x + (double)c1.y * xb.y +
                  (double)c2.x * xc.x + (double)c2.y * xc.y;
            a1 += (double)d0.x * xa.x + (double)d0.y * xa.y + (double)d1.x * xb.x + (double)d1.y * xb.y +
                  (double)d2.x * xc.x + (double)d2.y * xc.y;
        }
    }
#pragma unroll
    for (int o = 2; o > 0; o >>= 1) {
        a0 += __shfl_down_sync(0xffffffffu, a0, o, 4);
        if (BS == 2) a1 += __shfl_down_sync(0xffffffffu, a1, o, 4);
    }
    if (ok && lane == 0) {
        if (BS == 1) {
            y[i] = (areal)((b ? (double)b[i] : 0.0) + alpha * a0);
        } else {
            y[2 * (int64_t)i] = (areal)((b ? (double)b[2 * (int64_t)i] : 0.0) + alpha * a0);
            y[2 * (int64_t)i + 1] = (areal)((b ? (double)b[2 * (int64_t)i + 1] : 0.0) + alpha * a1);
        }
    }
}

int hemo_bsr_spmv_ex(hemo_ctx* ctx, int bs, int n, const int32_t* rowptr, const int32_t* col, const areal* val,
                     const areal* x, double alpha, const areal* b, areal* y) {
    const int grid = hemo_grid((int64_t)n * 4, 256);
    if (bs == 1) k_bsr_spmv<1><<<grid, 256, 0, ctx->stream>>>(n, rowptr, col, val, x, alpha, b, y);
    else k_bsr_spmv<2><<<grid, 256, 0, ctx->stream>>>(n, rowptr, col, val, x, alpha, b, y);
    HEMO_LAUNCH_CHECK(ctx);
    return 0;
}

int hemo_bsr_spmv(hemo_ctx* ctx, int bs, int n, const int32_t* rowptr, const int32_t* col, const areal* val,
                  const areal* x, areal* y) {
    return hemo_bsr_spmv_ex(ctx, bs, n, rowptr, col, val, x, 1.0, nullptr, y);
}

__global__ void k_axpy(int64_t n, double a, const double* __restrict__ x, double* __restrict__ y) {
    for (int64_t i = blockIdx.x * (int64_t)blockDim.x + threadIdx.x; i < n; i += (int64_t)gridDim.x * blockDim.x)
        y[i] = fma(a, x[i], y[i]);
}

__global__ void k_scale_copy(int64_t n, double a, const double* __restrict__ x, double* __restrict__ y) {
    for (int64_t i = blockIdx.x * (int64_t)blockDim.x + threadIdx.x; i < n; i += (int64_t)gridDim.x * blockDim.x)
        y[i] = a * x[i];
}

__global__ void k_scale_inv_dev(int64_t n, const double* __restrict__ s, const double* __restrict__ x,
                                double* __restrict__ y) {
    const double a = 1.0 / s[0];
    for (int64_t i = blockIdx.x * (int64_t)blockDim.x + threadIdx.x; i < n; i += (int64_t)gridDim.x * blockDim.x)
        y[i] = a * x[i];
}

__global__ void __launch_bounds__(RED_THREADS)
k_dot_partial(int64_t n, const double* __restrict__ x, const double* __restrict__ y, double* __restrict__ partial) {
    __shared__ double sh[32];
    double acc = 0.0;
    for (int64_t i = blockIdx.x * (int64_t)blockDim.x + threadIdx.x; i < n; i += (int64_t)gridDim.x * blockDim.x)
        acc = fma(x[i], y[i], acc);
    acc = block_sum(acc, sh);
    if (threadIdx.x == 0) partial[blockIdx.x] = acc;
// ... 167 lines not shown
    k_reduce_final<<<k, RED_THREADS, 0, ctx->stream>>>(g, ctx->red_partial, ctx->red_out, -1);
    HEMO_LAUNCH_CHECK(ctx);
    HEMO_CHECK_CUDA(ctx, cudaMemcpyAsync(ctx->red_host, ctx->red_out, sizeof(double) * k, cudaMemcpyDeviceToHost, ctx->stream));
    HEMO_CHECK_CUDA(ctx, cudaStreamSynchronize(ctx->stream));
    for (int i = 0; i < k; ++i) h_host[i] = ctx->red_host[i];
    return 0;
}

int hemo_maxpy(hemo_ctx* ctx, int64_t n, int k, const double* V, int64_t ldv, const double* hcoef_dev, double sign,
               double* w, double* norm_host) {
    int rc = hemo_ensure_reduce(ctx, (size_t)RED_BLOCKS * 2, 512);
    if (rc) return rc;
    const int g = grid_for(n);
    HEMO_PROF_BEGIN(ctx, HEMO_PROF_MAXPY);
    k_maxpy_norm<<<g, RED_THREADS, sizeof(double) * (k > 0 ? k : 1), ctx->stream>>>(
        n, k, V, ldv, hcoef_dev, sign, w, norm_host ? ctx->red_partial : nullptr);
    HEMO_LAUNCH_CHECK(ctx);
    HEMO_PROF_END(ctx, HEMO_PROF_MAXPY);
    if (norm_host) {
        k_reduce_final<<<1, RED_THREADS, 0, ctx->stream>>>(g, ctx->red_partial, ctx->red_out + 500, 0);
        HEMO_LAUNCH_CHECK(ctx);
        HEMO_CHECK_CUDA(ctx, cudaMemcpyAsync(ctx->red_host + 500, ctx->red_out + 500, sizeof(double),
                                             cudaMemcpyDeviceToHost, ctx->stream));
        HEMO_CHECK_CUDA(ctx, cudaStreamSynchronize(ctx->stream));
        *norm_host = ctx->red_host[500];
    }
    return 0;
}

__global__ void __launch_bounds__(RED_THREADS)
k_sub_mean_partials(int64_t n, int nparts, const double* __restrict__ partial, double* __restrict__ x) {
    __shared__ double sh[32];
    __shared__ double mean;
    double acc = 0.0;
    for (int t = threadIdx.x; t < nparts; t += blockDim.x) acc += partial[t];
    acc = block_sum(acc, sh);
    if (threadIdx.x == 0) mean = acc / (double)n;
    __syncthreads();
    const double m = mean;
    for (int64_t i = blockIdx.x * (int64_t)blockDim.x + threadIdx.x; i < n; i += (int64_t)gridDim.x * blockDim.x)
        x[i] -= m;
}

__global__ void __launch_bounds__(RED_THREADS)
k_sum_partial(int64_t n, const double* src, double* dst, double* __restrict__ partial) {
    __shared__ double sh[32];
    double acc = 0.0;
    for (int64_t i = blockIdx.x * (int64_t)blockDim.x + threadIdx.x; i < n; i += (int64_t)gridDim.x * blockDim.x) {
        const double v = src[i];
        if (dst != src) dst[i] = v;
        acc += v;
    }
    acc = block_sum(acc, sh);
    if (threadIdx.x == 0) partial[blockIdx.x] = acc;
}

int hemo_copy_remove_mean(hemo_ctx* ctx, int64_t n, const double* src, double* x) {
    int rc = hemo_ensure_reduce(ctx, (size_t)RED_BLOCKS * 2, 512);
    if (rc) return rc;
    const int g = grid_for(n);
    k_sum_partial<<<g, RED_THREADS, 0, ctx->stream>>>(n, src, x, ctx->red_partial);
    HEMO_LAUNCH_CHECK(ctx);
    k_sub_mean_partials<<<g, RED_THREADS, 0, ctx->stream>>>(n, g, ctx->red_partial, x);
    HEMO_LAUNCH_CHECK(ctx);
    return 0;
}

int hemo_remove_mean(hemo_ctx* ctx, int64_t n, double* x) { return hemo_copy_remove_mean(ctx, n, x, x); }
```

### cfd_hemodynamic_b200/csrc/solver.cu

```cuda
#include <math.h>

#include "hemo_internal.cuh"

int hemo_spmv_block(hemo_ctx* ctx, int rows, int cols, const double* vals, const double* xu, const double* xp,
                    double alpha, const double* bu, const double* bp, double* yu, double* yp);
int hemo_scale_copy(hemo_ctx* ctx, int64_t n, double a, const double* x, double* y);
int hemo_mdot(hemo_ctx* ctx, int64_t n, int k, const double* V, int64_t ldv, const double* w, double* h_host);
int hemo_maxpy(hemo_ctx* ctx, int64_t n, int k, const double* V, int64_t ldv, const double* hcoef_dev, double sign,
               double* w, double* norm_host);
int hemo_remove_mean(hemo_ctx* ctx, int64_t n, double* x);
int hemo_copy_remove_mean(hemo_ctx* ctx, int64_t n, const double* src, double* x);
int hemo_amg_numeric_shift(hemo_ctx* ctx, HemoAmg* amg, double coarse_shift);

__global__ void __launch_bounds__(256)
k_extract_a00(int64_t nnz_node, const int32_t* __restrict__ nrowptr, const int32_t* __restrict__ rowof,
              const int32_t* __restrict__ ncol, const uint8_t* __restrict__ mask,
              const double* __restrict__ vals, areal* __restrict__ out, areal2* __restrict__ a01) {
    const int64_t s = blockIdx.x * (int64_t)blockDim.x + threadIdx.x;
    if (s >= nnz_node) return;
    const int i = rowof[s];
    {
        const int r0 = nrowptr[i];
        const int deg = nrowptr[i + 1] - r0;
        const int t = (int)(s - r0);
        const int64_t ru0 = 6 * (int64_t)r0, ru1 = ru0 + 3 * deg;
        areal2 g;
        g.x = (areal)vals[ru0 + 2 * deg + t];
        g.y = (areal)vals[ru1 + 2 * deg + t];
        a01[s] = g;
    }
    if (mask) {
        const int j = ncol[s];
        if (mask[i] || mask[j]) {
// ... 8 lines not shown
    const int r0 = nrowptr[i];
    const int deg = nrowptr[i + 1] - r0;
    const int t = (int)(s - r0);
    const int64_t ru0 = 6 * (int64_t)r0, ru1 = ru0 + 3 * deg;
    areal2 a, b;
    a.x = (areal)vals[ru0 + 2 * t]; a.y = (areal)vals[ru0 + 2 * t + 1];
    b.x = (areal)vals[ru1 + 2 * t]; b.y = (areal)vals[ru1 + 2 * t + 1];
    reinterpret_cast<areal2*>(out)[2 * s] = a;
    reinterpret_cast<areal2*>(out)[2 * s + 1] = b;
}

__global__ void __launch_bounds__(256)
k_lap_with_bc(int n, int64_t nnz_node, const int32_t* __restrict__ rowof, const int32_t* __restrict__ ncol,
              const double* __restrict__ lap, const uint8_t* __restrict__ dofflag ,
              areal* __restrict__ out) {
    const int64_t s = blockIdx.x * (int64_t)blockDim.x + threadIdx.x;
    if (s >= nnz_node) return;
    double v = lap[s];
    if (dofflag) {
        const int i = rowof[s], j = ncol[s];
        const bool fi = dofflag[i] != 0, fj = dofflag[j] != 0;
        if (fi || fj) v = (i == j) ? 1.0 : 0.0;
    }
    out[s] = (areal)v;
}

__global__ void k_areal_to_double(int64_t n, const areal* __restrict__ x, double* __restrict__ y) {
    const int64_t i = blockIdx.x * (int64_t)blockDim.x + threadIdx.x;
    if (i < n) y[i] = (double)x[i];
}

__global__ void k_mask_nodes(int n, int bs, const uint8_t* __restrict__ mask, double* __restrict__ x) {
    const int i = blockIdx.x * blockDim.x + threadIdx.x;
    if (i >= n || !mask[i]) return;
    for (int k = 0; k < bs; ++k) x[(int64_t)i * bs + k] = 0.0;
}

__global__ void __launch_bounds__(256)
k_a01_residual(int n, const int32_t* __restrict__ nrowptr, const int32_t* __restrict__ ncol,
               const areal2* __restrict__ a01, const double* __restrict__ zp, const double* __restrict__ ru,
               double* __restrict__ tu) {
    const int gt = blockIdx.x * blockDim.x + threadIdx.x;
    const int i = gt >> 2, lane = gt & 3;
    const bool ok = i < n;
    const int r0 = ok ? nrowptr[i] : 0, r1 = ok ? nrowptr[i + 1] : 0;
    double a0 = 0.0, a1 = 0.0;
    for (int s = r0 + lane; s < r1; s += 4) {
        const areal2 g = a01[s];
        const double z = zp[ncol[s]];
        a0 = fma((double)g.x, z, a0);
        a1 = fma((double)g.y, z, a1);
    }
#pragma unroll
    for (int o = 2; o > 0; o >>= 1) {
        a0 += __shfl_down_sync(0xffffffffu, a0, o, 4);
        a1 += __shfl_down_sync(0xffffffffu, a1, o, 4);
    }
    if (ok && lane == 0) {
        tu[2 * (int64_t)i] = ru[2 * (int64_t)i] - a0;
        tu[2 * (int64_t)i + 1] = ru[2 * (int64_t)i + 1] - a1;
    }
}

__global__ void __launch_bounds__(256)
k_a01_residual_row(int n, const int32_t* __restrict__ nrowptr, const int32_t* __restrict__ ncol,
                   const areal2* __restrict__ a01, const double* __restrict__ zp, const double* __restrict__ ru,
                   double* __restrict__ tu) {
    const int i = blockIdx.x * blockDim.x + threadIdx.x;
    if (i >= n) return;
    const int r0 = nrowptr[i], r1 = nrowptr[i + 1];
    double a0 = 0.0, a1 = 0.0;
    for (int s = r0; s < r1; s += 4) {
        int t[4], j[4];
        areal2 g[4];
        double z[4];
#pragma unroll
        for (int u = 0; u < 4; ++u) t[u] = s + u < r1 ? s + u : r1 - 1;
#pragma unroll
        for (int u = 0; u < 4; ++u) j[u] = ncol[t[u]];
#pragma unroll
        for (int u = 0; u < 4; ++u) g[u] = a01[t[u]];
        __syncwarp(__activemask());
#pragma unroll
        for (int u = 0; u < 4; ++u) z[u] = zp[j[u]];
        __syncwarp(__activemask());
#pragma unroll
        for (int u = 0; u < 4; ++u) {
            const double m = s + u < r1 ? z[u] : 0.0;
            a0 = fma((double)g[u].x, m, a0);
            a1 = fma((double)g[u].y, m, a1);
        }
    }
    tu[2 * (int64_t)i] = ru[2 * (int64_t)i] - a0;
    tu[2 * (int64_t)i + 1] = ru[2 * (int64_t)i + 1] - a1;
}

__global__ void __launch_bounds__(256)
k_node_spmv_scalar(int n, const int32_t* __restrict__ nrowptr, const int32_t* __restrict__ ncol,
                   const areal* __restrict__ val, const double* __restrict__ q, double* __restrict__ out) {
    const int gt = blockIdx.x * blockDim.x + threadIdx.x;
    const int i = gt >> 2, lane = gt & 3;
    const bool ok = i < n;
    const int r0 = ok ? nrowptr[i] : 0, r1 = ok ? nrowptr[i + 1] : 0;
    double a = 0.0;
    for (int s = r0 + lane; s < r1; s += 4) a = fma((double)val[s], q[ncol[s]], a);
    a += __shfl_down_sync(0xffffffffu, a, 2, 4);
    a += __shfl_down_sync(0xffffffffu, a, 1, 4);
    if (ok && lane == 0) out[i] = a;
}

__global__ void k_schur_combine(int n, double cm, double cl, double cc, const double* __restrict__ tp,
                                const double* __restrict__ mass, const double* __restrict__ qp,
                                const double* __restrict__ conv, const uint8_t* __restrict__ dofflag ,
                                const double* __restrict__ rp, double* __restrict__ zp) {
    const int i = blockIdx.x * blockDim.x + threadIdx.x;
    if (i >= n) return;
    double v = cm * tp[i] / mass[i] + cl * qp[i];
    if (conv) v += cc * conv[i] / mass[i];
    if (dofflag && dofflag[i]) v = rp[i];
    zp[i] = v;
}

static int pc_build_graph(hemo_ctx* ctx, const double* vals_dev);

template <bool ADD>
__global__ void __launch_bounds__(256)
k_csr_apply_d(int nrows, const int32_t* __restrict__ rowptr, const int32_t* __restrict__ col, const double* __restrict__ val,
              const double* __restrict__ x, double scale, double* __restrict__ y) {
    const int gt = blockIdx.x * blockDim.x + threadIdx.x;
    const int i = gt >> 2, lane = gt & 3;
    const bool ok = i < nrows;
    const int r0 = ok ? rowptr[i] : 0, r1 = ok ? rowptr[i + 1] : 0;
    double a = 0.0;
    for (int t = r0 + lane; t < r1; t += 4) a = fma(val[t], x[col[t]], a);
    a += __shfl_xor_sync(0xffffffffu, a, 1, 4);
    a += __shfl_xor_sync(0xffffffffu, a, 2, 4);
    if (ok && lane == 0) y[i] = ADD ? y[i] + scale * a : scale * a;
}

extern "C" int hemo_pc_set_coarse_pressure(hemo_ctx* ctx, hemo_ctx* coarse_ctx, int coarse_n, const int32_t* p_rowptr,
                                           const int32_t* p_col, const double* p_val, const int32_t* r_rowptr,
                                           const int32_t* r_col, const double* r_val, int cycles) {
    if (!ctx) return HEMO_EINVAL;
    cudaFree(ctx->cp_rowptr); cudaFree(ctx->cp_col); cudaFree(ctx->cp_val);
    cudaFree(ctx->cr_rowptr); cudaFree(ctx->cr_col); cudaFree(ctx->cr_val);
    cudaFree(ctx->coarse_rhs); cudaFree(ctx->coarse_sol);
    ctx->cp_rowptr = ctx->cp_col = ctx->cr_rowptr = ctx->cr_col = nullptr;
    ctx->cp_val = ctx->cr_val = ctx->coarse_rhs = ctx->coarse_sol = nullptr;
// ... 14 lines not shown
    if ((rc = hemo_upload(ctx, &ctx->cr_rowptr, r_rowptr, (size_t)coarse_n + 1, false))) return rc;
    if ((rc = hemo_upload(ctx, &ctx->cr_col, r_col, (size_t)r_rowptr[coarse_n], false))) return rc;
    if ((rc = hemo_upload(ctx, &ctx->cr_val, r_val, (size_t)r_rowptr[coarse_n], false))) return rc;
    if ((rc = hemo_alloc(ctx, &ctx->coarse_rhs, (size_t)coarse_n))) return rc;
    if ((rc = hemo_alloc(ctx, &ctx->coarse_sol, (size_t)coarse_n))) return rc;
    HEMO_CHECK_CUDA(ctx, cudaStreamSynchronize(ctx->stream));
    ctx->coarse_ctx = coarse_ctx;
    ctx->coarse_n = coarse_n;
    ctx->coarse_cycles = cycles > 0 ? cycles : 1;
    return 0;
}

static int coarse_pressure_fork(hemo_ctx* ctx, const double* t_dev) {
    hemo_ctx* cc = ctx->coarse_ctx;
    const int nc = ctx->coarse_n;
    int rc = 0;
    if (!ctx->side_stream) {
        HEMO_CHECK_CUDA(ctx, cudaStreamCreateWithFlags(&ctx->side_stream, cudaStreamNonBlocking));
        HEMO_CHECK_CUDA(ctx, cudaEventCreateWithFlags(&ctx->ev_fork, cudaEventDisableTiming));
        HEMO_CHECK_CUDA(ctx, cudaEventCreateWithFlags(&ctx->ev_join, cudaEventDisableTiming));
    }
    cudaStream_t main_st = ctx->stream, side = ctx->side_stream;
    HEMO_CHECK_CUDA(ctx, cudaEventRecord(ctx->ev_fork, main_st));
    HEMO_CHECK_CUDA(ctx, cudaStreamWaitEvent(side, ctx->ev_fork, 0));
    ctx->stream = side;
    do {
        k_csr_apply_d<false><<<hemo_grid((int64_t)nc * 4, 256), 256, 0, side>>>(nc, ctx->cr_rowptr, ctx->cr_col, ctx->cr_val, t_dev,
                                                                               1.0, ctx->coarse_rhs);
        ctx->launches++;
        if (cudaGetLastError() != cudaSuccess) { rc = HEMO_ESTATE; ctx->err = "coarse restriction launch failed"; break; }
        if ((rc = hemo_comm_allreduce_j(ctx, ctx->coarse_rhs, nc))) break;
        cudaStream_t saved = cc->stream;
        const bool saved_cap = cc->capturing;
        const int64_t before = cc->launches;
        cc->stream = side;
        cc->capturing = ctx->capturing;
        cc->opts.cheb_degree = ctx->opts.cheb_degree;
        cc->opts.cheb_degree_pre = ctx->opts.cheb_degree_pre;
        cc->opts.cheb_ratio = ctx->opts.cheb_ratio;
        rc = hemo_amg_vcycle(cc, &cc->amg[1], ctx->coarse_rhs, ctx->coarse_sol, ctx->coarse_cycles);
        ctx->launches += cc->launches - before;
        cc->stream = saved;
        cc->capturing = saved_cap;
        if (rc) ctx->err = cc->err;
    } while (0);
    ctx->stream = main_st;
    if (rc) return rc;
    HEMO_CHECK_CUDA(ctx, cudaEventRecord(ctx->ev_join, side));
    return 0;
}

static int coarse_pressure_join(hemo_ctx* ctx, double* q_dev) {
    const int n = ctx->n;
    cudaStream_t st = ctx->stream;
    HEMO_CHECK_CUDA(ctx, cudaStreamWaitEvent(st, ctx->ev_join, 0));
    k_csr_apply_d<true><<<hemo_grid((int64_t)n * 4, 256), 256, 0, st>>>(n, ctx->cp_rowptr, ctx->cp_col, ctx->cp_val, ctx->coarse_sol,
                                                                       1.0, q_dev);
    HEMO_LAUNCH_CHECK(ctx);
    return 0;
}

static inline const uint8_t* pressure_flags(const hemo_ctx* ctx) {
    return ctx->have_bc ? ctx->dofflag + (size_t)ctx->dim * ctx->n : nullptr;
}

extern "C" int hemo_remove_mean_vec(hemo_ctx* ctx, int64_t n, double* x_dev) {
    if (!ctx || !x_dev || n <= 0) return HEMO_EINVAL;
    return hemo_remove_mean(ctx, n, x_dev);
}

extern "C" int hemo_set_external_schur(hemo_ctx* ctx, int on) {
    if (!ctx) return HEMO_EINVAL;
    ctx->external_schur = on != 0;
    return 0;
}

// ... 148 lines not shown
    amg.apply_b = b_dev; amg.apply_x = x_dev; amg.apply_cycles = ncycles; amg.apply_valid = true;
    HEMO_CHECK_CUDA(ctx, cudaGraphLaunch(amg.apply_exec, st));
    ctx->launches += amg.apply_nodes;
    return 0;
}

extern "C" int hemo_amg_get_level_values(hemo_ctx* ctx, int which, int level, double* vals_dev, int64_t capacity) {
    if (!ctx || which < 0 || which > 1 || !vals_dev) return HEMO_EINVAL;
    HemoAmg& amg = ctx->amg[which];
    if (!amg.ready || level < 0 || level >= amg.nlev) return HEMO_EINVAL;
    const int64_t cnt = amg.op[level].nnzb * amg.bs * amg.bs;
    if (capacity < cnt) return HEMO_EINVAL;
    k_areal_to_double<<<hemo_grid(cnt, 256), 256, 0, ctx->stream>>>(cnt, amg.op[level].val, vals_dev);
    HEMO_LAUNCH_CHECK(ctx);
    return 0;
}

int hemo_pc_apply_body(hemo_ctx* ctx, const double* vals_dev, const double* r_dev, double* z_dev) {
    const int n = ctx->n;
    cudaStream_t st = ctx->stream;
    const double* ru = r_dev;
    const double* rp = r_dev + ctx->dim * (int64_t)n;
    double* zu = z_dev;
    double* zp = z_dev + ctx->dim * (int64_t)n;
    double* tp = ctx->pc_tmp_p;
    double* qp = ctx->pc_tmp_p2;
    double* tu = ctx->pc_tmp_u;
    int rc;
    if (!ctx->external_schur) {
    if (ctx->opts.project_pressure && !ctx->pc_mask) {
        if ((rc = hemo_copy_remove_mean(ctx, n, rp, tp))) return rc;
    } else {
        HEMO_CHECK_CUDA(ctx, cudaMemcpyAsync(tp, rp, sizeof(double) * n, cudaMemcpyDeviceToDevice, st));
        if (ctx->pc_mask) {
            k_mask_nodes<<<hemo_grid(n, 256), 256, 0, st>>>(n, 1, ctx->pc_mask, tp);
            HEMO_LAUNCH_CHECK(ctx);
        }
        if (ctx->opts.project_pressure && (rc = hemo_remove_mean(ctx, n, tp))) return rc;
    }
    if (ctx->coarse_ctx && (rc = coarse_pressure_fork(ctx, tp))) return rc;
    if ((rc = hemo_amg_vcycle(ctx, &ctx->amg[1], tp, qp, ctx->opts.amg_cycles_p))) return rc;
    if (ctx->coarse_ctx) {
        HEMO_PROF_BEGIN(ctx, HEMO_PROF_COARSE);
        if ((rc = coarse_pressure_join(ctx, qp))) return rc;
        HEMO_PROF_END(ctx, HEMO_PROF_COARSE);
    }
    const bool pcd = ctx->npconv_coef != 0.0 && ctx->npconv;
    if (pcd) {
        k_node_spmv_scalar<<<hemo_grid((int64_t)n * 4, 256), 256, 0, st>>>(n, ctx->nrowptr, ctx->ncol, ctx->npconv, qp,
                                                                          ctx->pc_tmp_u2);
        HEMO_LAUNCH_CHECK(ctx);
    }
    k_schur_combine<<<hemo_grid(n, 256), 256, 0, st>>>(n, ctx->opts.schur_mass_coef, ctx->opts.schur_lap_coef,
                                                       ctx->npconv_coef, tp, ctx->mass, qp,
                                                       pcd ? ctx->pc_tmp_u2 : nullptr, pressure_flags(ctx), rp, zp);
    HEMO_LAUNCH_CHECK(ctx);
    if (ctx->opts.project_pressure && (rc = hemo_remove_mean(ctx, n, zp))) return rc;
    }
    if (ctx->dim == 3)
        return hemo_tet_velocity_solve(ctx, vals_dev, ru, zp, tu, ctx->pc_tmp_u2, zu, 4 * ctx->opts.amg_cycles_u, 2.0 / 3.0);
    if (n >= 32768 && ctx->nnz_node <= 12 * (int64_t)n)
        k_a01_residual_row<<<hemo_grid(n, 256), 256, 0, st>>>(n, ctx->nrowptr, ctx->ncol, ctx->a01, zp, ru, tu);
    else
        k_a01_residual<<<hemo_grid((int64_t)n * 4, 256), 256, 0, st>>>(n, ctx->nrowptr, ctx->ncol, ctx->a01, zp, ru, tu);
    HEMO_LAUNCH_CHECK(ctx);
    if (ctx->pc_mask) {
        k_mask_nodes<<<hemo_grid(n, 256), 256, 0, st>>>(n, 2, ctx->pc_mask, tu);
        HEMO_LAUNCH_CHECK(ctx);
    }
    if ((rc = hemo_amg_vcycle(ctx, &ctx->amg[0], tu, zu, ctx->opts.amg_cycles_u))) return rc;
    return 0;
}

static int pc_build_graph(hemo_ctx* ctx, const double* vals_dev) {
    if (!ctx->use_graph || ctx->stream == 0) return 0;
    cudaStream_t st = ctx->stream;
    int rc = hemo_ensure_reduce(ctx, (size_t)1184 * 8, 512);
    if (rc) return rc;
    HEMO_CHECK_CUDA(ctx, cudaStreamSynchronize(st));
    const int64_t before = ctx->launches;
    ctx->capturing = true;
    cudaError_t e = cudaStreamBeginCapture(st, cudaStreamCaptureModeThreadLocal);
    if (e != cudaSuccess) {
        ctx->capturing = false;
        cudaGetLastError();
        ctx->use_graph = 0;
        return 0;
    }
    rc = hemo_pc_apply_body(ctx, vals_dev, ctx->pc_in, ctx->pc_out);
    cudaGraph_t g = nullptr;
    e = cudaStreamEndCapture(st, &g);
    ctx->capturing = false;
    ctx->pc_graph_nodes = ctx->launches - before;
    ctx->launches = before;
    if (rc != 0 || e != cudaSuccess || !g) {
        cudaGetLastError();
        if (g) cudaGraphDestroy(g);
        if (rc == HEMO_ERETRY) return pc_build_graph(ctx, vals_dev);
        ctx->use_graph = 0;
        if (rc) return rc;
        return 0;
    }
// ... 21 lines not shown
        const size_t bytes = sizeof(double) * (size_t)(ctx->dim + 1) * (size_t)ctx->n;
        cudaStream_t st = ctx->stream;
        HEMO_CHECK_CUDA(ctx, cudaMemcpyAsync(ctx->pc_in, r_dev, bytes, cudaMemcpyDeviceToDevice, st));
        if (ctx->external_schur)
            HEMO_CHECK_CUDA(ctx, cudaMemcpyAsync(ctx->pc_out + (size_t)ctx->dim * ctx->n, z_dev + (size_t)ctx->dim * ctx->n,
                                                 sizeof(double) * ctx->n, cudaMemcpyDeviceToDevice, st));
        HEMO_CHECK_CUDA(ctx, cudaGraphLaunch(ctx->pc_graph_exec, st));
        HEMO_CHECK_CUDA(ctx, cudaMemcpyAsync(z_dev, ctx->pc_out, bytes, cudaMemcpyDeviceToDevice, st));
        ctx->launches += ctx->pc_graph_nodes;
        return 0;
    }
    return hemo_pc_apply_body(ctx, vals_dev, r_dev, z_dev);
}

extern "C" int hemo_ctx_create(int device, hemo_ctx** out) {
    if (!out) return HEMO_EINVAL;
    cudaError_t e = cudaSetDevice(device);
    if (e != cudaSuccess) return (int)e;
    hemo_ctx* ctx = new hemo_ctx();
    ctx->device = device;
    ctx->opts.restart = 60;
    ctx->opts.max_it = 1000;
    ctx->opts.rtol = 1e-5;
    ctx->opts.atol = 1e-50;
    ctx->opts.amg_cycles_u = 1;
    ctx->opts.amg_cycles_p = 1;
    ctx->opts.cheb_degree = 2;
    ctx->opts.project_pressure = 0;
    ctx->opts.pc_mode = 0;
    ctx->opts.schur_mass_coef = 0.0;
    ctx->opts.schur_lap_coef = 1.0;
    ctx->opts.cheb_ratio = 4.0;
    ctx->opts.cheb_degree_pre = 0;
    *out = ctx;
    return 0;
}

extern "C" int hemo_ctx_destroy(hemo_ctx* ctx) {
    if (!ctx) return HEMO_EINVAL;
    cudaSetDevice(ctx->device);
    cudaFree(ctx->cellpos); cudaFree(ctx->mseg_ptr); cudaFree(ctx->mseg_src); cudaFree(ctx->vseg_ptr);
    cudaFree(ctx->vseg_src); cudaFree(ctx->diagslot); cudaFree(ctx->rowof); cudaFree(ctx->Ae); cudaFree(ctx->Fe);
    cudaFree(ctx->dvec); cudaFree(ctx->dofflag); cudaFree(ctx->dofmult); cudaFree(ctx->cellflag);
    for (int s = 0; s < HEMO_MAX_FACET_SETS; ++s) { cudaFree(ctx->fsets[s].cells); cudaFree(ctx->fsets[s].mask); }
    cudaFree(ctx->red_partial); cudaFree(ctx->red_out);
    if (ctx->red_host) cudaFreeHost(ctx->red_host);
    hemo_amg_free(&ctx->amg[0]); hemo_amg_free(&ctx->amg[1]);
    if (ctx->pc_graph_exec) cudaGraphExecDestroy(ctx->pc_graph_exec);
    if (ctx->pc_graph) cudaGraphDestroy(ctx->pc_graph);
    cudaFree(ctx->npconv); cudaFree(ctx->schur_mask); cudaFree(ctx->schur_tmp);
    cudaFree(ctx->wss_cell2t); cudaFree(ctx->wss_tmp);
    free(ctx->qrules);
    free(ctx->p2rules);
    hemo_tet_free(ctx);
    hemo_cc_free(ctx);
    cudaFree(ctx->pc_in); cudaFree(ctx->pc_out); cudaFree(ctx->pc_mask); cudaFree(ctx->kry_coef); cudaFree(ctx->a01);
    cudaFree(ctx->pc_tmp_u); cudaFree(ctx->pc_tmp_u2); cudaFree(ctx->pc_tmp_p); cudaFree(ctx->pc_tmp_p2);
    cudaFree(ctx->kry_V); cudaFree(ctx->kry_Z); cudaFree(ctx->kry_w);
    cudaFree(ctx->cp_rowptr); cudaFree(ctx->cp_col); cudaFree(ctx->cp_val);
    cudaFree(ctx->cr_rowptr); cudaFree(ctx->cr_col); cudaFree(ctx->cr_val);
    cudaFree(ctx->coarse_rhs); cudaFree(ctx->coarse_sol);
    if (ctx->side_stream) cudaStreamDestroy(ctx->side_stream);
    if (ctx->ev_fork) cudaEventDestroy(ctx->ev_fork);
    if (ctx->ev_join) cudaEventDestroy(ctx->ev_join);
    hemo_krylov_free(ctx);
    hemo_comm_free(ctx);
// ... 37 lines not shown
```

### include/hemo.h

```cpp
#ifndef HEMO_H
#define HEMO_H

#include <stdint.h>

#ifdef __cplusplus
extern "C" {
#endif

typedef struct hemo_ctx hemo_ctx;

#define HEMO_OK 0
#define HEMO_EINVAL (-1)
#define HEMO_ESTATE (-2)
#define HEMO_DIVERGED (-100)

typedef struct hemo_params {
    double dt, rho, mu;
    double f[2];
    double eps0;
} hemo_params;

typedef struct hemo_facet_coef {
    double a_p, pconst, a_g, a_s, a_n, beta_n, a_b, beta_b;
} hemo_facet_coef;
// ... 96 lines not shown
int hemo_mask_nodes(hemo_ctx* ctx, const uint8_t* node_mask_dev, double* x_dev);
int hemo_vec_mdot(hemo_ctx* ctx, int64_t n, int k, const double* V_dev, int64_t ldv, const double* w_dev,
                  double* h_host);
int hemo_vec_maxpy(hemo_ctx* ctx, int64_t n, int k, const double* V_dev, int64_t ldv,
                   const double* coef_host, double sign, double* w_dev, double* normsq_host);
int hemo_vec_scale(hemo_ctx* ctx, int64_t n, double a, const double* x_dev, double* y_dev);

int hemo_comm_unique_id(char* out128);
int hemo_comm_init(hemo_ctx* ctx, const char* uid128, int rank, int nranks);
int hemo_comm_info(hemo_ctx* ctx, int* rank, int* nranks, int* nccl_version, int64_t* halo_updates,
                   int64_t* allreduces);
int hemo_comm_set_partition(hemo_ctx* ctx, int n_owned, int nneigh, const int32_t* peers_host,
                            const int32_t* send_ptr_host, const int32_t* send_nodes_host,
                            const int32_t* recv_ptr_host, int ras_overlap);
int hemo_set_graph(hemo_ctx* ctx, int n, const int32_t* rowptr_dev, const int32_t* col_dev, int64_t nnz);
int hemo_pc_set_coarse_pressure(hemo_ctx* ctx, hemo_ctx* coarse_ctx, int coarse_n, const int32_t* p_rowptr,
                                const int32_t* p_col, const double* p_val, const int32_t* r_rowptr,
                                const int32_t* r_col, const double* r_val, int cycles);
int hemo_comm_halo_update(hemo_ctx* ctx, double* v_dev);
int hemo_comm_allreduce(hemo_ctx* ctx, double* buf_dev, int count);
int hemo_global_dot(hemo_ctx* ctx, const double* x_dev, const double* y_dev, double* out_host);
int hemo_set_poll_interval(hemo_ctx* ctx, int every);

int hemo_use_graph(hemo_ctx* ctx, int on);
int hemo_set_schur_mask(hemo_ctx* ctx, const uint8_t* node_mask_dev);
int hemo_pc_set_schur_operator(hemo_ctx* ctx, const double* x_dev, const double* un_dev,
                               const double* vals_dev, double c_u, double coarse_shift);
int hemo_amg_set_fine_pattern(hemo_ctx* ctx, int which, const int32_t* rowptr_host, const int32_t* col_host);
int hemo_pc_set_schur_selfp(hemo_ctx* ctx, const double* vals_dev, double coarse_shift);
int hemo_pc_set_convection(hemo_ctx* ctx, const double* x_dev, const double* un_dev, double coef);
int hemo_pc_apply(hemo_ctx* ctx, const double* vals_dev, const double* r_dev, double* z_dev);
int hemo_fgmres(hemo_ctx* ctx, const double* vals_dev, const double* b_dev, double* y_dev,
                int* its_out, double* rel_resid_out);

#ifdef __cplusplus
}
#endif
#endif
```

Measured before the change: 46.48 million.

## Enable programmatic dependent launch across solver kernels with prologue prefetch

Adds programmatic dependent launch (griddepcontrol wait/trigger) to the many small AMG, Chebyshev, SpMV and Schur kernels, and launches them through a HEMO_LAUNCH wrapper, on by default and switchable off with HEMO_PDL. Kernels are restructured so loads that do not depend on the previous kernel (row pointers, column indices, matrix values, dinv) are issued before the wait, overlapping them with the tail of the prior kernel. This targets launch latency and inter-kernel gaps in the latency-bound Krylov/AMG loop. The cost is more complex kernel code and a risk of reading data before the dependency is satisfied if any prefetched operand is actually written upstream.

```diff
diff --git a/cfd_hemodynamic_b200/_lib.py b/cfd_hemodynamic_b200/_lib.py
--- a/cfd_hemodynamic_b200/_lib.py
+++ b/cfd_hemodynamic_b200/_lib.py
@@ -109,6 +109,7 @@
     "hemo_comm_allreduce": (_I, [_VP, _VP, _I]),
     "hemo_global_dot": (_I, [_VP, _VP, _VP, C.POINTER(_D)]),
     "hemo_set_poll_interval": (_I, [_VP, _I]),
+    "hemo_krylov_graph_info": (_I, [_VP, C.POINTER(_L), C.POINTER(_L)]),
 }
 
 _lib = None
@@ -437,6 +438,11 @@
     def pc_apply(self, vals, r, z):
         self._check(self.lib.hemo_pc_apply(self._ctx, _ptr(vals), _ptr(r), _ptr(z)), "hemo_pc_apply")
 
+    def krylov_graph_info(self):
+        nodes, edges = C.c_int64(), C.c_int64()
+        self._check(self.lib.hemo_krylov_graph_info(self._ctx, C.byref(nodes), C.byref(edges)), "hemo_krylov_graph_info")
+        return nodes.value, edges.value
+
     @staticmethod
     def comm_unique_id() -> bytes:
         buf = C.create_string_buffer(128)
diff --git a/cfd_hemodynamic_b200/csrc/amg.cu b/cfd_hemodynamic_b200/csrc/amg.cu
--- a/cfd_hemodynamic_b200/csrc/amg.cu
+++ b/cfd_hemodynamic_b200/csrc/amg.cu
@@ -250,16 +250,22 @@
 
 __global__ void k_axpy_areal(int64_t n, double a, const areal* __restrict__ x, areal* __restrict__ y) {
     const int64_t i = blockIdx.x * (int64_t)blockDim.x + threadIdx.x;
+    hemo_pdl_wait();
+    hemo_pdl_trigger();
     if (i < n) y[i] = (areal)fma(a, (double)x[i], (double)y[i]);
 }
 
 __global__ void k_to_areal(int64_t n, const double* __restrict__ x, areal* __restrict__ y) {
     const int64_t i = blockIdx.x * (int64_t)blockDim.x + threadIdx.x;
+    hemo_pdl_wait();
+    hemo_pdl_trigger();
     if (i < n) y[i] = (areal)x[i];
 }
 
 __global__ void k_from_areal(int64_t n, const areal* __restrict__ x, double* __restrict__ y) {
     const int64_t i = blockIdx.x * (int64_t)blockDim.x + threadIdx.x;
+    hemo_pdl_wait();
+    hemo_pdl_trigger();
     if (i < n) y[i] = (double)x[i];
 }
 
@@ -268,6 +274,8 @@
                                   double inv_theta, areal* __restrict__ r, areal* __restrict__ d,
                                   areal* __restrict__ x) {
     const int64_t i = blockIdx.x * (int64_t)blockDim.x + threadIdx.x;
+    hemo_pdl_wait();
+    hemo_pdl_trigger();
     if (i >= N) return;
     const double rv = dinv[i] * b[i];
     r[i] = rv;
@@ -277,34 +285,47 @@
 }
 
 template <int BS>
-__device__ __forceinline__ void row_product(const int32_t* __restrict__ rowptr, const int32_t* __restrict__ col,
-                                            const areal* __restrict__ val, const areal* __restrict__ x,
-                                            int i, bool ok, int lane, double acc[BS]) {
-#pragma unroll
-    for (int k = 0; k < BS; ++k) acc[k] = 0.0;
-    const int r0 = ok ? rowptr[i] : 0, r1 = ok ? rowptr[i + 1] : 0;
-    for (int t = r0 + lane; t < r1; t += 12) {
+struct CsrChunk {
+    int j0, j1, j2;
+    areal2 a0, a1, a2, b0, b1, b2;
+    areal v0, v1, v2;
+    __device__ __forceinline__ void load(const int32_t* __restrict__ col, const areal* __restrict__ val, int t, int r1) {
         const int t1 = t + 4, t2 = t + 8;
         const bool p1 = t1 < r1, p2 = t2 < r1;
-        const int j0 = col[t];
-        const int j1 = p1 ? col[t1] : j0;
-        const int j2 = p2 ? col[t2] : j0;
+        j0 = col[t];
+        j1 = p1 ? col[t1] : j0;
+        j2 = p2 ? col[t2] : j0;
         if (BS == 1) {
-            const double v0 = (double)val[t], x0 = (double)x[j0];
-            const double v1 = p1 ? (double)val[t1] : 0.0, x1 = (double)x[j1];
-            const double v2 = p2 ? (double)val[t2] : 0.0, x2 = (double)x[j2];
-            acc[0] = fma(v0, x0, acc[0]);
-            acc[0] = fma(v1, x1, acc[0]);
-            acc[0] = fma(v2, x2, acc[0]);
+            v0 = val[t];
+            v1 = p1 ? val[t1] : (areal)0;
+            v2 = p2 ? val[t2] : (areal)0;
         } else {
             const areal2* v2p = reinterpret_cast<const areal2*>(val);
-            const areal2* x2p = reinterpret_cast<const areal2*>(x);
-            const areal2 a0 = v2p[2 * (int64_t)t], b0 = v2p[2 * (int64_t)t + 1], xa = x2p[j0];
-            areal2 a1, b1, a2, b2;
+            a0 = v2p[2 * (int64_t)t]; b0 = v2p[2 * (int64_t)t + 1];
             a1.x = a1.y = b1.x = b1.y = a2.x = a2.y = b2.x = b2.y = 0;
             if (p1) { a1 = v2p[2 * (int64_t)t1]; b1 = v2p[2 * (int64_t)t1 + 1]; }
             if (p2) { a2 = v2p[2 * (int64_t)t2]; b2 = v2p[2 * (int64_t)t2 + 1]; }
-            const areal2 xb = x2p[j1], xc = x2p[j2];
+        }
+    }
+};
+
+template <int BS>
+__device__ __forceinline__ void row_product(const int32_t* __restrict__ col, const areal* __restrict__ val,
+                                            const areal* __restrict__ x, int r0, int r1, int lane, CsrChunk<BS>& ch,
+                                            double acc[BS]) {
+#pragma unroll
+    for (int k = 0; k < BS; ++k) acc[k] = 0.0;
+    for (int t = r0 + lane; t < r1; t += 12) {
+        if (t != r0 + lane) ch.load(col, val, t, r1);
+        if (BS == 1) {
+            const double x0 = (double)x[ch.j0], x1 = (double)x[ch.j1], x2 = (double)x[ch.j2];
+            acc[0] = fma((double)ch.v0, x0, acc[0]);
+            acc[0] = fma((double)ch.v1, x1, acc[0]);
+            acc[0] = fma((double)ch.v2, x2, acc[0]);
+        } else {
+            const areal2* x2p = reinterpret_cast<const areal2*>(x);
+            const areal2 xa = x2p[ch.j0], xb = x2p[ch.j1], xc = x2p[ch.j2];
+            const areal2 a0 = ch.a0, a1 = ch.a1, a2 = ch.a2, b0 = ch.b0, b1 = ch.b1, b2 = ch.b2;
             acc[0] += (double)a0.x * xa.x + (double)a0.y * xa.y + (double)a1.x * xb.x + (double)a1.y * xb.y +
                       (double)a2.x * xc.x + (double)a2.y * xc.y;
             acc[BS - 1] += (double)b0.x * xa.x + (double)b0.y * xa.y + (double)b1.x * xb.x + (double)b1.y * xb.y +
@@ -326,8 +347,13 @@
     const int gt = blockIdx.x * blockDim.x + threadIdx.x;
     const int i = gt >> 2, lane = gt & 3;
     const bool ok = i < n;
+    const int r0 = ok ? rowptr[i] : 0, r1 = ok ? rowptr[i + 1] : 0;
+    CsrChunk<BS> ch;
+    if (r0 + lane < r1) ch.load(col, val, r0 + lane, r1);
+    hemo_pdl_wait();
+    hemo_pdl_trigger();
     double acc[BS];
-    row_product<BS>(rowptr, col, val, xin, i, ok, lane, acc);
+    row_product<BS>(col, val, xin, r0, r1, lane, ch, acc);
     if (ok && lane < BS) {
         const int64_t q = (int64_t)i * BS + lane;
         const double rv = dinv[q] * (b[q] - (lane == 0 ? acc[0] : acc[BS - 1]));
@@ -345,29 +371,48 @@
     const int i = gt >> 2, lane = gt & 3;
     const bool ok = i < n;
     const int r0 = ok ? rowptr[i] : 0, r1 = ok ? rowptr[i + 1] : 0;
+    int j0 = 0, j1 = 0;
+    areal2 a0, b0, a1, b1;
+    areal v0 = 0, v1 = 0;
+    areal d[2 * BS];
+    auto fetch = [&](int t) {
+        const int t1 = t + 4;
+        const bool p1 = t1 < r1;
+        j0 = col[t];
+        j1 = p1 ? col[t1] : j0;
+        if (BS == 1) {
+            v0 = val[t];
+            v1 = p1 ? val[t1] : (areal)0;
+        } else {
+            const areal2* v2p = reinterpret_cast<const areal2*>(val);
+            a0 = v2p[2 * (int64_t)t]; b0 = v2p[2 * (int64_t)t + 1];
+            a1.x = a1.y = b1.x = b1.y = 0;
+            if (p1) { a1 = v2p[2 * (int64_t)t1]; b1 = v2p[2 * (int64_t)t1 + 1]; }
+        }
+#pragma unroll
+        for (int k = 0; k < BS; ++k) {
+            d[k] = dinv[(int64_t)j0 * BS + k];
+            d[BS + k] = dinv[(int64_t)j1 * BS + k];
+        }
+    };
+    if (r0 + lane < r1) fetch(r0 + lane);
+    hemo_pdl_wait();
+    hemo_pdl_trigger();
     double acc[BS];
 #pragma unroll
     for (int k = 0; k < BS; ++k) acc[k] = 0.0;
     for (int t = r0 + lane; t < r1; t += 8) {
-        const int t1 = t + 4;
-        const bool p1 = t1 < r1;
-        const int j0 = col[t];
-        const int j1 = p1 ? col[t1] : j0;
+        if (t != r0 + lane) fetch(t);
         if (BS == 1) {
-            const double x0 = (double)dinv[j0] * (double)b[j0] * inv_theta;
-            const double x1 = (double)dinv[j1] * (double)b[j1] * inv_theta;
-            acc[0] = fma((double)val[t], x0, acc[0]);
-            acc[0] = fma(p1 ? (double)val[t1] : 0.0, x1, acc[0]);
+            const double x0 = (double)d[0] * (double)b[j0] * inv_theta;
+            const double x1 = (double)d[BS] * (double)b[j1] * inv_theta;
+            acc[0] = fma((double)v0, x0, acc[0]);
+            acc[0] = fma((double)v1, x1, acc[0]);
         } else {
-            const areal2* v2p = reinterpret_cast<const areal2*>(val);
-            const areal2 a0 = v2p[2 * (int64_t)t], b0 = v2p[2 * (int64_t)t + 1];
-            areal2 a1, b1;
-            a1.x = a1.y = b1.x = b1.y = 0;
-            if (p1) { a1 = v2p[2 * (int64_t)t1]; b1 = v2p[2 * (int64_t)t1 + 1]; }
-            const double xa0 = (double)dinv[2 * (int64_t)j0] * (double)b[2 * (int64_t)j0] * inv_theta;
-            const double xa1 = (double)dinv[2 * (int64_t)j0 + 1] * (double)b[2 * (int64_t)j0 + 1] * inv_theta;
-            const double xb0 = (double)dinv[2 * (int64_t)j1] * (double)b[2 * (int64_t)j1] * inv_theta;
-            const double xb1 = (double)dinv[2 * (int64_t)j1 + 1] * (double)b[2 * (int64_t)j1 + 1] * inv_theta;
+            const double xa0 = (double)d[0] * (double)b[2 * (int64_t)j0] * inv_theta;
+            const double xa1 = (double)d[1] * (double)b[2 * (int64_t)j0 + 1] * inv_theta;
+            const double xb0 = (double)d[BS] * (double)b[2 * (int64_t)j1] * inv_theta;
+            const double xb1 = (double)d[BS + 1] * (double)b[2 * (int64_t)j1 + 1] * inv_theta;
             acc[0] += (double)a0.x * xa0 + (double)a0.y * xa1 + (double)a1.x * xb0 + (double)a1.y * xb1;
             acc[BS - 1] += (double)b0.x * xa0 + (double)b0.y * xa1 + (double)b1.x * xb0 + (double)b1.y * xb1;
         }
@@ -395,8 +440,13 @@
     const int gt = blockIdx.x * blockDim.x + threadIdx.x;
     const int i = gt >> 2, lane = gt & 3;
     const bool ok = i < n;
+    const int r0 = ok ? rowptr[i] : 0, r1 = ok ? rowptr[i + 1] : 0;
+    CsrChunk<BS> ch;
+    if (r0 + lane < r1) ch.load(col, val, r0 + lane, r1);
+    hemo_pdl_wait();
+    hemo_pdl_trigger();
     double acc[BS];
-    row_product<BS>(rowptr, col, val, dold, i, ok, lane, acc);
+    row_product<BS>(col, val, dold, r0, r1, lane, ch, acc);
     if (ok && lane < BS) {
         const int64_t q = (int64_t)i * BS + lane;
         const double rv = r[q] - dinv[q] * (lane == 0 ? acc[0] : acc[BS - 1]);
@@ -478,47 +528,64 @@
     }
 };
 
-template <int BS, typename XF>
-__device__ __forceinline__ void sell_row_product(const int32_t* __restrict__ sptr, const int32_t* __restrict__ scol,
-                                                 const areal* __restrict__ sval, int i, const XF xf, double acc[BS]) {
+template <int BS>
+struct SellRow {
     typedef typename std::conditional<BS == 1, areal, areal4>::type blk;
-#pragma unroll
-    for (int k = 0; k < BS; ++k) acc[k] = 0.0;
-    const int s = i >> 5, lane = i & 31;
-    const int base = sptr[s];
-    const int W = (sptr[s + 1] - base) >> 5;
-    const int32_t* __restrict__ c = scol + base + lane;
-    const blk* __restrict__ v = reinterpret_cast<const blk*>(sval) + base + lane;
-    for (int k = 0; k < W; k += 4) {
+    const int32_t* __restrict__ c;
+    const blk* __restrict__ v;
+    int W;
+    bool group;
+    int j[4];
+    blk a[4];
+    template <bool GROUP>
+    __device__ __forceinline__ void begin(const int32_t* __restrict__ sptr, const int32_t* __restrict__ scol,
+                                          const areal* __restrict__ sval, int i) {
+        const int s = i >> 5, lane = i & 31;
+        const int base = sptr[s];
+        W = (sptr[s + 1] - base) >> 5;
+        c = scol + base + lane;
+        v = reinterpret_cast<const blk*>(sval) + base + lane;
+        group = GROUP;
+        if (GROUP && W > 0) fetch(0);
+    }
+    __device__ __forceinline__ void fetch(int k) {
         int kk[4];
-        bool ok[4];
-#pragma unroll
-        for (int u = 0; u < 4; ++u) { ok[u] = k + u < W; kk[u] = 32 * (ok[u] ? k + u : W - 1); }
-        int j[4];
-        blk a[4];
-        typename XF::raw xr[4];
+#pragma unroll
+        for (int u = 0; u < 4; ++u) kk[u] = 32 * (k + u < W ? k + u : W - 1);
 #pragma unroll
         for (int u = 0; u < 4; ++u) j[u] = ldg_nc(c + kk[u]);
 #pragma unroll
         for (int u = 0; u < 4; ++u) a[u] = ldg_nc(v + kk[u]);
-        __syncwarp();
-#pragma unroll
-        for (int u = 0; u < 4; ++u) xr[u] = xf.load(j[u]);
-        __syncwarp();
-#pragma unroll
-        for (int u = 0; u < 4; ++u) {
-            double xv[BS];
-            xf.value(xr[u], xv);
-            if constexpr (BS == 1) {
-                acc[0] = fma(ok[u] ? (double)a[u] : 0.0, xv[0], acc[0]);
-            } else {
-                const double m = ok[u] ? 1.0 : 0.0;
-                acc[0] += m * ((double)a[u].x * xv[0] + (double)a[u].y * xv[1]);
-                acc[1] += m * ((double)a[u].z * xv[0] + (double)a[u].w * xv[1]);
+    }
+    template <typename XF>
+    __device__ __forceinline__ void product(const XF xf, double acc[BS]) {
+#pragma unroll
+        for (int k = 0; k < BS; ++k) acc[k] = 0.0;
+        for (int k = 0; k < W; k += 4) {
+            bool ok[4];
+#pragma unroll
+            for (int u = 0; u < 4; ++u) ok[u] = k + u < W;
+            if (k > 0 || !group) fetch(k);
+            typename XF::raw xr[4];
+            __syncwarp();
+#pragma unroll
+            for (int u = 0; u < 4; ++u) xr[u] = xf.load(j[u]);
+            __syncwarp();
+#pragma unroll
+            for (int u = 0; u < 4; ++u) {
+                double xv[BS];
+                xf.value(xr[u], xv);
+                if constexpr (BS == 1) {
+                    acc[0] = fma(ok[u] ? (double)a[u] : 0.0, xv[0], acc[0]);
+                } else {
+                    const double m = ok[u] ? 1.0 : 0.0;
+                    acc[0] += m * ((double)a[u].x * xv[0] + (double)a[u].y * xv[1]);
+                    acc[1] += m * ((double)a[u].z * xv[0] + (double)a[u].w * xv[1]);
+                }
             }
         }
     }
-}
+};
 
 template <int BS>
 __global__ void __launch_bounds__(256)
@@ -526,9 +593,13 @@
                   const areal* __restrict__ dinv, const areal* __restrict__ b, double inv_theta,
                   const areal* __restrict__ xin, areal* __restrict__ r, areal* __restrict__ d) {
     const int i = blockIdx.x * blockDim.x + threadIdx.x;
+    SellRow<BS> row;
+    if (i < n) row.template begin<true>(sptr, scol, sval, i);
+    hemo_pdl_wait();
+    hemo_pdl_trigger();
     if (i >= n) return;
     double acc[BS];
-    sell_row_product<BS>(sptr, scol, sval, i, VecLoad<BS>{xin}, acc);
+    row.product(VecLoad<BS>{xin}, acc);
 #pragma unroll
     for (int k = 0; k < BS; ++k) {
         const int64_t q = (int64_t)i * BS + k;
@@ -544,9 +615,13 @@
                           const areal* __restrict__ sval, const areal* __restrict__ dinv, const TB* __restrict__ b,
                           double inv_theta, areal* __restrict__ x, areal* __restrict__ r, areal* __restrict__ bcopy) {
     const int i = blockIdx.x * blockDim.x + threadIdx.x;
+    hemo_pdl_wait();
+    hemo_pdl_trigger();
     if (i >= n) return;
+    SellRow<BS> row;
+    row.template begin<false>(sptr, scol, sval, i);
     double acc[BS];
-    sell_row_product<BS>(sptr, scol, sval, i, JacobiLoad<BS, TB>{dinv, b, inv_theta}, acc);
+    row.product(JacobiLoad<BS, TB>{dinv, b, inv_theta}, acc);
 #pragma unroll
     for (int k = 0; k < BS; ++k) {
         const int64_t q = (int64_t)i * BS + k;
@@ -564,9 +639,13 @@
                  areal* __restrict__ dnew, areal* __restrict__ r, areal* __restrict__ x, int add_old,
                  double* __restrict__ x64) {
     const int i = blockIdx.x * blockDim.x + threadIdx.x;
+    SellRow<BS> row;
+    if (i < n) row.template begin<true>(sptr, scol, sval, i);
+    hemo_pdl_wait();
+    hemo_pdl_trigger();
     if (i >= n) return;
     double acc[BS];
-    sell_row_product<BS>(sptr, scol, sval, i, VecLoad<BS>{dold}, acc);
+    row.product(VecLoad<BS>{dold}, acc);
 #pragma unroll
     for (int k = 0; k < BS; ++k) {
         const int64_t q = (int64_t)i * BS + k;
@@ -586,9 +665,13 @@
 k_sell_residual(int n, const int32_t* __restrict__ sptr, const int32_t* __restrict__ scol, const areal* __restrict__ sval,
                 const areal* __restrict__ x, const areal* __restrict__ b, areal* __restrict__ y) {
     const int i = blockIdx.x * blockDim.x + threadIdx.x;
+    SellRow<BS> row;
+    if (i < n) row.template begin<true>(sptr, scol, sval, i);
+    hemo_pdl_wait();
+    hemo_pdl_trigger();
     if (i >= n) return;
     double acc[BS];
-    sell_row_product<BS>(sptr, scol, sval, i, VecLoad<BS>{x}, acc);
+    row.product(VecLoad<BS>{x}, acc);
 #pragma unroll
     for (int k = 0; k < BS; ++k) {
         const int64_t q = (int64_t)i * BS + k;
@@ -628,14 +711,19 @@
 k_prolong_add_row(int nrows, const int32_t* __restrict__ rowptr, const int32_t* __restrict__ col,
                   const double* __restrict__ w, const areal* __restrict__ x, areal* __restrict__ y) {
     const int i = blockIdx.x * blockDim.x + threadIdx.x;
-    if (i >= nrows) return;
-    const int r0 = rowptr[i], r1 = rowptr[i + 1];
+    const bool ok = i < nrows;
+    const int r0 = ok ? rowptr[i] : 0, r1 = ok ? rowptr[i + 1] : 0;
+    int j = 0;
+    double wt = 0.0;
+    if (r0 < r1) { j = col[r0]; wt = w[r0]; }
+    hemo_pdl_wait();
+    hemo_pdl_trigger();
+    if (!ok) return;
     double acc[BS];
 #pragma unroll
     for (int k = 0; k < BS; ++k) acc[k] = 0.0;
     for (int t = r0; t < r1; ++t) {
-        const int j = col[t];
-        const double wt = w[t];
+        if (t != r0) { j = col[t]; wt = w[t]; }
 #pragma unroll
         for (int k = 0; k < BS; ++k) acc[k] = fma(wt, (double)x[(int64_t)j * BS + k], acc[k]);
     }
@@ -654,16 +742,24 @@
     const int I = gt >> 2, lane = gt & 3;
     const bool ok = I < nrows;
     const int r0 = ok ? rowptr[I] : 0, r1 = ok ? rowptr[I + 1] : 0;
+    int j0 = 0, j1 = 0, j2 = 0;
+    double w0 = 0.0, w1 = 0.0, w2 = 0.0;
+    auto fetch = [&](int t) {
+        const int t1 = t + 4, t2 = t + 8;
+        const bool p1 = t1 < r1, p2 = t2 < r1;
+        j0 = col[t];
+        j1 = p1 ? col[t1] : j0;
+        j2 = p2 ? col[t2] : j0;
+        w0 = w[t]; w1 = p1 ? w[t1] : 0.0; w2 = p2 ? w[t2] : 0.0;
+    };
+    if (r0 + lane < r1) fetch(r0 + lane);
+    hemo_pdl_wait();
+    hemo_pdl_trigger();
     double acc[BS];
 #pragma unroll
     for (int k = 0; k < BS; ++k) acc[k] = 0.0;
     for (int t = r0 + lane; t < r1; t += 12) {
-        const int t1 = t + 4, t2 = t + 8;
-        const bool p1 = t1 < r1, p2 = t2 < r1;
-        const int j0 = col[t];
-        const int j1 = p1 ? col[t1] : j0;
-        const int j2 = p2 ? col[t2] : j0;
-        const double w0 = w[t], w1 = p1 ? w[t1] : 0.0, w2 = p2 ? w[t2] : 0.0;
+        if (t != r0 + lane) fetch(t);
 #pragma unroll
         for (int k = 0; k < BS; ++k) {
             const double x0 = (double)x[(int64_t)j0 * BS + k], x1 = (double)x[(int64_t)j1 * BS + k],
@@ -887,6 +983,8 @@
 __global__ void __launch_bounds__(1024)
 k_coarse_vcycle(const HemoCoarseLevel* __restrict__ desc, int nl, const areal* __restrict__ b0, areal* __restrict__ x0,
                 int degree_pre, int degree, double ratio, const double* __restrict__ dense_inv, int dense_n) {
+    hemo_pdl_wait();
+    hemo_pdl_trigger();
     CtaScope sc;
     coarse_vcycle_body<BS>(sc, desc, nl, b0, x0, degree_pre, degree, ratio, dense_inv, dense_n);
 }
@@ -964,6 +1062,8 @@
 k_dense_gemv(int N, const double* __restrict__ inv, const areal* __restrict__ b, areal* __restrict__ y) {
     const int row = (blockIdx.x * blockDim.x + threadIdx.x) >> 5;
     const int lane = threadIdx.x & 31;
+    hemo_pdl_wait();
+    hemo_pdl_trigger();
     double acc = 0.0;
     if (row < N)
         for (int c = lane; c < N; c += 32) acc += inv[(int64_t)row * N + c] * b[c];
@@ -1319,15 +1419,14 @@
     areal* d0 = A.d;
     areal* d1 = A.d + N;
     if (x_is_zero) {
-        k_cheb_start_zero<BS><<<hemo_grid(N, 256), 256, 0, st>>>(N, A.dinv, b, 1.0 / theta, A.r, d0, x);
+        HEMO_LAUNCH(ctx, k_cheb_start_zero<BS>, hemo_grid(N, 256), 256, 0, st, N, A.dinv, b, 1.0 / theta, A.r, d0, x);
     } else if (A.sell_ptr) {
-        k_sell_cheb_start<BS><<<hemo_grid(A.n, 256), 256, 0, st>>>(A.n, A.sell_ptr, A.sell_col, A.sell_val, A.dinv, b, 1.0 / theta,
-                                                                    x, A.r, d0);
+        HEMO_LAUNCH(ctx, k_sell_cheb_start<BS>, hemo_grid(A.n, 256), 256, 0, st, A.n, A.sell_ptr, A.sell_col, A.sell_val, A.dinv, b,
+                    1.0 / theta, x, A.r, d0);
     } else {
-        k_cheb_start<BS><<<hemo_grid((int64_t)A.n * 4, 256), 256, 0, st>>>(A.n, A.rowptr, A.col, A.val, A.dinv, b, 1.0 / theta, x,
-                                                              A.r, d0);
-    }
-    HEMO_LAUNCH_CHECK(ctx);
+        HEMO_LAUNCH(ctx, k_cheb_start<BS>, hemo_grid((int64_t)A.n * 4, 256), 256, 0, st, A.n, A.rowptr, A.col, A.val, A.dinv, b,
+                    1.0 / theta, x, A.r, d0);
+    }
     bool pending = !x_is_zero;
     for (int k = 1; k < degree; ++k) {
         const double rho_new = 1.0 / (2.0 * sigma - rho);
@@ -1336,22 +1435,18 @@
         if (fine) HEMO_PROF_BEGIN(ctx, BS == 2 ? HEMO_PROF_CHEB_U0 : HEMO_PROF_CHEB_P0);
         const bool last = (k == degree - 1);
         if (A.sell_ptr)
-            k_sell_cheb_step<BS><<<hemo_grid(A.n, 256), 256, 0, st>>>(A.n, A.sell_ptr, A.sell_col, A.sell_val, A.dinv, c1, c2, d0, d1,
-                                                                       A.r, x, pending ? 1 : 0, last ? x64 : nullptr);
+            HEMO_LAUNCH(ctx, k_sell_cheb_step<BS>, hemo_grid(A.n, 256), 256, 0, st, A.n, A.sell_ptr, A.sell_col, A.sell_val, A.dinv, c1,
+                        c2, d0, d1, A.r, x, pending ? 1 : 0, last ? x64 : nullptr);
         else
-            k_cheb_step<BS><<<hemo_grid((int64_t)A.n * 4, 256), 256, 0, st>>>(A.n, A.rowptr, A.col, A.val, A.dinv, c1, c2, d0, d1, A.r, x,
-                                                                 pending ? 1 : 0, last ? x64 : nullptr);
+            HEMO_LAUNCH(ctx, k_cheb_step<BS>, hemo_grid((int64_t)A.n * 4, 256), 256, 0, st, A.n, A.rowptr, A.col, A.val, A.dinv, c1, c2,
+                        d0, d1, A.r, x, pending ? 1 : 0, last ? x64 : nullptr);
         if (last && x64 && wrote64) *wrote64 = true;
-        HEMO_LAUNCH_CHECK(ctx);
         if (fine) HEMO_PROF_END(ctx, BS == 2 ? HEMO_PROF_CHEB_U0 : HEMO_PROF_CHEB_P0);
         pending = false;
         areal* t = d0; d0 = d1; d1 = t;
         rho = rho_new;
     }
-    if (pending) {
-        k_axpy_areal<<<hemo_grid(N, 256), 256, 0, st>>>(N, 1.0, d0, x);
-        HEMO_LAUNCH_CHECK(ctx);
-    }
+    if (pending) HEMO_LAUNCH(ctx, k_axpy_areal, hemo_grid(N, 256), 256, 0, st, N, 1.0, d0, x);
     return 0;
 }
 
@@ -1394,15 +1489,13 @@
         return 0;
     }
     if (l == amg->fuse_level) {
-        k_coarse_vcycle<BS><<<1, 1024, 0, st>>>(amg->fuse_desc + (l - amg->fuse_base), amg->nlev - l, b, x, degree_pre, degree, ratio,
-                                                amg->dense_inv, amg->dense_n);
-        HEMO_LAUNCH_CHECK(ctx);
+        HEMO_LAUNCH(ctx, k_coarse_vcycle<BS>, 1, 1024, 0, st, amg->fuse_desc + (l - amg->fuse_base), amg->nlev - l, b, x, degree_pre,
+                    degree, ratio, amg->dense_inv, amg->dense_n);
         return 0;
     }
     if (l == amg->nlev - 1) {
         const int N = amg->dense_n;
-        k_dense_gemv<<<hemo_grid((int64_t)N * 32, 256), 256, 0, st>>>(N, amg->dense_inv, b, x);
-        HEMO_LAUNCH_CHECK(ctx);
+        HEMO_LAUNCH(ctx, k_dense_gemv, hemo_grid((int64_t)N * 32, 256), 256, 0, st, N, amg->dense_inv, b, x);
         return 0;
     }
     int rc;
@@ -1410,38 +1503,37 @@
         const double lmax = A.lmax, lmin = lmax / ratio;
         const double inv_theta = 1.0 / (0.5 * (lmax + lmin));
         const int g = hemo_grid((int64_t)A.n * 4, 256);
+        areal* const no_copy = nullptr;
         if (A.sell_ptr) {
             const int gs = hemo_grid(A.n, 256);
-            if (b64) k_sell_presmooth_residual<BS, double><<<gs, 256, 0, st>>>(A.n, A.sell_ptr, A.sell_col, A.sell_val, A.dinv, b64,
-                                                                                inv_theta, x, A.r, const_cast<areal*>(b));
-            else k_sell_presmooth_residual<BS, areal><<<gs, 256, 0, st>>>(A.n, A.sell_ptr, A.sell_col, A.sell_val, A.dinv, b,
-                                                                          inv_theta, x, A.r, nullptr);
-        } else if (b64) k_presmooth_residual<BS, double><<<g, 256, 0, st>>>(A.n, A.rowptr, A.col, A.val, A.dinv, b64, inv_theta, x, A.r,
-                                                                      const_cast<areal*>(b));
-        else k_presmooth_residual<BS, areal><<<g, 256, 0, st>>>(A.n, A.rowptr, A.col, A.val, A.dinv, b, inv_theta, x, A.r, nullptr);
-        HEMO_LAUNCH_CHECK(ctx);
+            if (b64) HEMO_LAUNCH(ctx, (k_sell_presmooth_residual<BS, double>), gs, 256, 0, st, A.n, A.sell_ptr, A.sell_col, A.sell_val,
+                                 A.dinv, b64, inv_theta, x, A.r, const_cast<areal*>(b));
+            else HEMO_LAUNCH(ctx, (k_sell_presmooth_residual<BS, areal>), gs, 256, 0, st, A.n, A.sell_ptr, A.sell_col, A.sell_val, A.dinv,
+                             b, inv_theta, x, A.r, no_copy);
+        } else if (b64) HEMO_LAUNCH(ctx, (k_presmooth_residual<BS, double>), g, 256, 0, st, A.n, A.rowptr, A.col, A.val, A.dinv, b64,
+                                    inv_theta, x, A.r, const_cast<areal*>(b));
+        else HEMO_LAUNCH(ctx, (k_presmooth_residual<BS, areal>), g, 256, 0, st, A.n, A.rowptr, A.col, A.val, A.dinv, b, inv_theta, x,
+                         A.r, no_copy);
     } else {
         if (b64) {
             const int64_t N = (int64_t)A.n * BS;
-            k_to_areal<<<hemo_grid(N, 256), 256, 0, st>>>(N, b64, const_cast<areal*>(b));
-            HEMO_LAUNCH_CHECK(ctx);
+            HEMO_LAUNCH(ctx, k_to_areal, hemo_grid(N, 256), 256, 0, st, N, b64, const_cast<areal*>(b));
         }
         if ((rc = smooth_t<BS>(ctx, A, b, x, x_is_zero, degree_pre, ratio))) return rc;
         if (A.sell_ptr) {
-            k_sell_residual<BS><<<hemo_grid(A.n, 256), 256, 0, st>>>(A.n, A.sell_ptr, A.sell_col, A.sell_val, x, b, A.r);
-            HEMO_LAUNCH_CHECK(ctx);
+            HEMO_LAUNCH(ctx, k_sell_residual<BS>, hemo_grid(A.n, 256), 256, 0, st, A.n, A.sell_ptr, A.sell_col, A.sell_val, x, b, A.r);
         } else if ((rc = hemo_bsr_spmv_ex(ctx, BS, A.n, A.rowptr, A.col, A.val, x, -1.0, b, A.r))) return rc;
     }
     const HemoAmgLevel& L = amg->lev[l];
     HemoAmgOp& C = amg->op[l + 1];
-    k_transfer<BS, false><<<hemo_grid((int64_t)C.n * 4, 256), 256, 0, st>>>(C.n, L.r_rowptr, L.r_col, L.r_val, A.r, C.b);
-    HEMO_LAUNCH_CHECK(ctx);
+    HEMO_LAUNCH(ctx, (k_transfer<BS, false>), hemo_grid((int64_t)C.n * 4, 256), 256, 0, st, C.n, L.r_rowptr, L.r_col, L.r_val, A.r,
+                C.b);
     if ((rc = vcycle_t<BS>(ctx, amg, l + 1, C.b, C.x, true))) return rc;
     if (L.nnz_p <= 6 * (int64_t)A.n && A.n >= 32768)
-        k_prolong_add_row<BS><<<hemo_grid(A.n, 256), 256, 0, st>>>(A.n, L.p_rowptr, L.p_col, L.p_val, C.x, x);
+        HEMO_LAUNCH(ctx, k_prolong_add_row<BS>, hemo_grid(A.n, 256), 256, 0, st, A.n, L.p_rowptr, L.p_col, L.p_val, C.x, x);
     else
-        k_transfer<BS, true><<<hemo_grid((int64_t)A.n * 4, 256), 256, 0, st>>>(A.n, L.p_rowptr, L.p_col, L.p_val, C.x, x);
-    HEMO_LAUNCH_CHECK(ctx);
+        HEMO_LAUNCH(ctx, (k_transfer<BS, true>), hemo_grid((int64_t)A.n * 4, 256), 256, 0, st, A.n, L.p_rowptr, L.p_col, L.p_val, C.x,
+                    x);
     if ((rc = smooth_t<BS>(ctx, A, b, x, false, degree, ratio, x64, wrote64))) return rc;
     return 0;
 }
@@ -1453,10 +1545,7 @@
     const int64_t N = (int64_t)top.n * amg->bs;
     const int nc = ncycles > 0 ? ncycles : 1;
     const bool per_level_top = amg->nlev > 1 && amg->fuse_level != 0 && !(amg->fuse_level_grid == 0 && amg->grid_blocks > 0);
-    if (!per_level_top) {
-        k_to_areal<<<hemo_grid(N, 256), 256, 0, ctx->stream>>>(N, b, top.b);
-        HEMO_LAUNCH_CHECK(ctx);
-    }
+    if (!per_level_top) HEMO_LAUNCH(ctx, k_to_areal, hemo_grid(N, 256), 256, 0, ctx->stream, N, b, top.b);
     bool wrote64 = false;
     for (int c = 0; c < nc; ++c) {
         const double* b64 = (per_level_top && c == 0) ? b : nullptr;
@@ -1465,9 +1554,6 @@
         else rc = vcycle_t<1>(ctx, amg, 0, top.b, top.x, c == 0, b64, x64, &wrote64);
         if (rc) return rc;
     }
-    if (!wrote64) {
-        k_from_areal<<<hemo_grid(N, 256), 256, 0, ctx->stream>>>(N, top.x, x);
-        HEMO_LAUNCH_CHECK(ctx);
-    }
+    if (!wrote64) HEMO_LAUNCH(ctx, k_from_areal, hemo_grid(N, 256), 256, 0, ctx->stream, N, top.x, x);
     return 0;
 }
diff --git a/cfd_hemodynamic_b200/csrc/comm.cu b/cfd_hemodynamic_b200/csrc/comm.cu
--- a/cfd_hemodynamic_b200/csrc/comm.cu
+++ b/cfd_hemodynamic_b200/csrc/comm.cu
@@ -102,6 +102,7 @@
         return 1000 + (int)r;
     }
     ctx->comm = c;
+    ctx->pdl = 0;
     return 0;
 }
 
diff --git a/cfd_hemodynamic_b200/csrc/hemo_internal.cuh b/cfd_hemodynamic_b200/csrc/hemo_internal.cuh
--- a/cfd_hemodynamic_b200/csrc/hemo_internal.cuh
+++ b/cfd_hemodynamic_b200/csrc/hemo_internal.cuh
@@ -140,6 +140,7 @@
     bool iter_valid = false;
     const double* iter_vals = nullptr;
     int64_t iter_nodes = 0;
+    int64_t iter_kernel_nodes = 0, iter_prog_edges = 0;
 };
 
 struct hemo_ctx {
@@ -152,6 +153,7 @@
     cudaStream_t stream = 0;
     std::string err;
     int64_t launches = 0;
+    int pdl = 1;
 
     int nv = 3;
     int dim = 2;
@@ -269,6 +271,62 @@
                          cudaGetErrorString(_e) + " at " + __FILE__ + ":" + std::to_string(__LINE__); \
             return (int)_e;                                          \
         }                                                            \
+    } while (0)
+
+__device__ __forceinline__ void hemo_pdl_wait() {
+#if defined(__CUDA_ARCH__) && __CUDA_ARCH__ >= 900
+    asm volatile("griddepcontrol.wait;" ::: "memory");
+#endif
+}
+__device__ __forceinline__ void hemo_pdl_trigger() {
+#if defined(__CUDA_ARCH__) && __CUDA_ARCH__ >= 900
+    asm volatile("griddepcontrol.launch_dependents;" ::: "memory");
+#endif
+}
+
+static inline bool hemo_pdl_allowed(cudaStream_t st) {
+    if (st == 0) return false;
+    cudaStreamCaptureStatus cs;
+    const cudaGraphNode_t* deps = nullptr;
+    size_t nd = 0;
+    if (cudaStreamGetCaptureInfo(st, &cs, nullptr, nullptr, &deps, &nd) != cudaSuccess) {
+        cudaGetLastError();
+        return false;
+    }
+    if (cs != cudaStreamCaptureStatusActive) return true;
+    cudaGraphNodeType t;
+    return nd == 1 && cudaGraphNodeGetType(deps[0], &t) == cudaSuccess && t == cudaGraphNodeTypeKernel;
+}
+
+template <typename... P, typename... A>
+static inline cudaError_t hemo_launch_kernel(hemo_ctx* ctx, void (*kernel)(P...), dim3 grid, dim3 block, size_t smem,
+                                             cudaStream_t st, A... args) {
+    cudaLaunchConfig_t cfg = {};
+    cfg.gridDim = grid;
+    cfg.blockDim = block;
+    cfg.dynamicSmemBytes = smem;
+    cfg.stream = st;
+    cudaLaunchAttribute at[1];
+    if (ctx->pdl && hemo_pdl_allowed(st)) {
+        at[0].id = cudaLaunchAttributeProgrammaticStreamSerialization;
+        at[0].val.programmaticStreamSerializationAllowed = 1;
+        cfg.attrs = at;
+        cfg.numAttrs = 1;
+    }
+    const cudaError_t e = cudaLaunchKernelEx(&cfg, kernel, args...);
+    const cudaError_t last = cudaGetLastError();
+    return e != cudaSuccess ? e : last;
+}
+
+#define HEMO_LAUNCH(ctx, kernel, grid, block, smem, st, ...)                                                        \
+    do {                                                                                                            \
+        (ctx)->launches++;                                                                                          \
+        cudaError_t _e = hemo_launch_kernel((ctx), kernel, dim3(grid), dim3(block), (size_t)(smem), (st), __VA_ARGS__); \
+        if (_e != cudaSuccess) {                                                                                    \
+            (ctx)->err = std::string("kernel launch: ") +                                                           \
+                         cudaGetErrorString(_e) + " at " + __FILE__ + ":" + std::to_string(__LINE__);              \
+            return (int)_e;                                                                                         \
+        }                                                                                                           \
     } while (0)
 
 static inline void hemo_prof_mark(hemo_ctx* ctx, int cls) {
diff --git a/cfd_hemodynamic_b200/csrc/krylov.cu b/cfd_hemodynamic_b200/csrc/krylov.cu
--- a/cfd_hemodynamic_b200/csrc/krylov.cu
+++ b/cfd_hemodynamic_b200/csrc/krylov.cu
@@ -106,6 +106,8 @@
 __global__ void __launch_bounds__(FG_THREADS)
 k_fg_load(const FgState* __restrict__ st, int64_t n, const double* __restrict__ V, int64_t ldv,
           const double* __restrict__ scale, double* __restrict__ pc_in) {
+    hemo_pdl_wait();
+    hemo_pdl_trigger();
     if (st->converged || st->cycle_full) return;
     const int j = st->j;
     const double s = scale[j];
@@ -118,12 +120,6 @@
 k_fg_spmv_node(const FgState* __restrict__ st, int n, int64_t nnz_node, const int32_t* __restrict__ nrowptr,
                const int32_t* __restrict__ ncol, const double* __restrict__ vals, const double* __restrict__ z,
                double* __restrict__ V, double* __restrict__ Z, int64_t ldv) {
-    if (st->converged || st->cycle_full) return;
-    const int j = st->j;
-    const double* xu = z;
-    const double* xp = z + 2 * (int64_t)n;
-    double* w = V + (int64_t)(j + 1) * ldv;
-    double* zj = Z + (int64_t)j * ldv;
     const int gt = blockIdx.x * blockDim.x + threadIdx.x;
     const int i = gt >> 3;
     const int lane = gt & 7;
@@ -131,14 +127,31 @@
     const int r0 = ok ? nrowptr[i] : 0;
     const int deg = ok ? nrowptr[i + 1] - r0 : 0;
     const int64_t ru0 = 6 * (int64_t)r0, ru1 = ru0 + 3 * deg, rp = 6 * nnz_node + 3 * (int64_t)r0;
+    int c = 0;
+    double v[9];
+    auto fetch = [&](int t) {
+        c = ncol[r0 + t];
+        v[0] = vals[ru0 + 2 * t]; v[1] = vals[ru0 + 2 * t + 1]; v[2] = vals[ru0 + 2 * deg + t];
+        v[3] = vals[ru1 + 2 * t]; v[4] = vals[ru1 + 2 * t + 1]; v[5] = vals[ru1 + 2 * deg + t];
+        v[6] = vals[rp + 2 * t];  v[7] = vals[rp + 2 * t + 1];  v[8] = vals[rp + 2 * deg + t];
+    };
+    if (lane < deg) fetch(lane);
+    hemo_pdl_wait();
+    hemo_pdl_trigger();
+    if (st->converged || st->cycle_full) return;
+    const int j = st->j;
+    const double* xu = z;
+    const double* xp = z + 2 * (int64_t)n;
+    double* w = V + (int64_t)(j + 1) * ldv;
+    double* zj = Z + (int64_t)j * ldv;
     double a0 = 0.0, a1 = 0.0, a2 = 0.0;
     for (int t = lane; t < deg; t += 8) {
-        const int c = ncol[r0 + t];
+        if (t != lane) fetch(t);
         const double2 xv = reinterpret_cast<const double2*>(xu)[c];
         const double x2 = xp[c];
-        a0 += vals[ru0 + 2 * t] * xv.x + vals[ru0 + 2 * t + 1] * xv.y + vals[ru0 + 2 * deg + t] * x2;
-        a1 += vals[ru1 + 2 * t] * xv.x + vals[ru1 + 2 * t + 1] * xv.y + vals[ru1 + 2 * deg + t] * x2;
-        a2 += vals[rp + 2 * t] * xv.x + vals[rp + 2 * t + 1] * xv.y + vals[rp + 2 * deg + t] * x2;
+        a0 += v[0] * xv.x + v[1] * xv.y + v[2] * x2;
+        a1 += v[3] * xv.x + v[4] * xv.y + v[5] * x2;
+        a2 += v[6] * xv.x + v[7] * xv.y + v[8] * x2;
     }
 #pragma unroll
     for (int o = 4; o > 0; o >>= 1) {
@@ -157,6 +170,8 @@
 __global__ void __launch_bounds__(FG_THREADS)
 k_fg_store(const FgState* __restrict__ st, int64_t n, const double* __restrict__ z, const double* __restrict__ w,
            double* __restrict__ V, double* __restrict__ Z, int64_t ldv) {
+    hemo_pdl_wait();
+    hemo_pdl_trigger();
     if (st->converged || st->cycle_full) return;
     const int j = st->j;
     double* wj = V + (int64_t)(j + 1) * ldv;
@@ -172,6 +187,8 @@
 k_fg_mdot(const FgState* __restrict__ st, FgSeg seg, const double* __restrict__ V, int64_t ldv,
           double* __restrict__ partial , int kpad) {
     extern __shared__ double acc_sh[];
+    hemo_pdl_wait();
+    hemo_pdl_trigger();
     if (st->converged || st->cycle_full) return;
     const int j = st->j, k = j + 1;
     const double* w = V + (int64_t)k * ldv;
@@ -234,6 +251,8 @@
 k_fg_mdot_final(const FgState* __restrict__ st, int nblk, const double* __restrict__ partial,
                 const double* __restrict__ scale, double* __restrict__ hcol) {
     __shared__ double sh[32];
+    hemo_pdl_wait();
+    hemo_pdl_trigger();
     if (st->converged || st->cycle_full) return;
     const int i = blockIdx.x;
     if (i > st->j) return;
@@ -294,6 +313,8 @@
            double* __restrict__ cs, double* __restrict__ sn, double* __restrict__ g, double* __restrict__ scale) {
     __shared__ double sh[32];
     extern __shared__ double hsh[];
+    hemo_pdl_wait();
+    hemo_pdl_trigger();
     if (st->converged || st->cycle_full) return;
     const int j = st->j, k = j + 1;
     double* w = V + (int64_t)k * ldv;
@@ -325,6 +346,8 @@
                             double* __restrict__ H, double* __restrict__ cs, double* __restrict__ sn,
                             double* __restrict__ g, double* __restrict__ scale) {
     extern __shared__ double gsh[];
+    hemo_pdl_wait();
+    hemo_pdl_trigger();
     if (st->converged || st->cycle_full) return;
     fg_givens(st, m, hcol, sqrt(fmax(normsq[0], 0.0)), H, cs, sn, g, scale, gsh);
 }
@@ -438,8 +461,7 @@
     cudaStream_t st = ctx->stream;
     const FgSeg seg = {K.seg_len0 ? K.seg_len0 : N, K.seg_off1, K.seg_len0 ? K.seg_len1 : 0};
     int rc;
-    k_fg_load<<<fg_grid(N, 4), FG_THREADS, 0, st>>>(p.st, N, ctx->kry_V, ldv, p.scale, ctx->pc_in);
-    HEMO_LAUNCH_CHECK(ctx);
+    HEMO_LAUNCH(ctx, k_fg_load, fg_grid(N, 4), FG_THREADS, 0, st, p.st, N, ctx->kry_V, ldv, p.scale, ctx->pc_in);
     if (ctx->comm && ctx->comm_ras_overlap && (rc = hemo_comm_halo(ctx, ctx->pc_in))) return rc;
     HEMO_PROF_BEGIN(ctx, HEMO_PROF_PC);
     if ((rc = hemo_pc_apply_body(ctx, vals_dev, ctx->pc_in, ctx->pc_out))) return rc;
@@ -448,12 +470,12 @@
     HEMO_PROF_BEGIN(ctx, HEMO_PROF_SPMV);
     if (ctx->dim == 3) {
         if ((rc = hemo_tet_spmv(ctx, vals_dev, ctx->pc_out, ctx->kry_w))) return rc;
-        k_fg_store<<<fg_grid(N, 4), FG_THREADS, 0, st>>>(p.st, N, ctx->pc_out, ctx->kry_w, ctx->kry_V, ctx->kry_Z, ldv);
+        HEMO_LAUNCH(ctx, k_fg_store, fg_grid(N, 4), FG_THREADS, 0, st, p.st, N, ctx->pc_out, ctx->kry_w, ctx->kry_V, ctx->kry_Z,
+                    ldv);
     } else {
-        k_fg_spmv_node<<<hemo_grid((int64_t)n * 8, 256), 256, 0, st>>>(p.st, n, ctx->nnz_node, ctx->nrowptr, ctx->ncol, vals_dev,
-                                                                    ctx->pc_out, ctx->kry_V, ctx->kry_Z, ldv);
-    }
-    HEMO_LAUNCH_CHECK(ctx);
+        HEMO_LAUNCH(ctx, k_fg_spmv_node, hemo_grid((int64_t)n * 8, 256), 256, 0, st, p.st, n, ctx->nnz_node, ctx->nrowptr,
+                    ctx->ncol, vals_dev, ctx->pc_out, ctx->kry_V, ctx->kry_Z, ldv);
+    }
     HEMO_PROF_END(ctx, HEMO_PROF_SPMV);
     const int64_t nown = seg.len0 + seg.len1;
     HEMO_PROF_BEGIN(ctx, HEMO_PROF_MDOT);
@@ -461,26 +483,44 @@
         const int kpad = m + 4;
         const int gm = fg_grid(nown, FG_TILE);
         const size_t smem = sizeof(double) * (FG_THREADS / 32) * kpad;
-        if (seg.len1 > 0) k_fg_mdot<true><<<gm, FG_THREADS, smem, st>>>(p.st, seg, ctx->kry_V, ldv, K.partial, kpad);
-        else k_fg_mdot<false><<<gm, FG_THREADS, smem, st>>>(p.st, seg, ctx->kry_V, ldv, K.partial, kpad);
-        HEMO_LAUNCH_CHECK(ctx);
-        k_fg_mdot_final<<<m, 128, 0, st>>>(p.st, gm, K.partial, p.scale, p.hcol);
-        HEMO_LAUNCH_CHECK(ctx);
+        if (seg.len1 > 0) HEMO_LAUNCH(ctx, k_fg_mdot<true>, gm, FG_THREADS, smem, st, p.st, seg, ctx->kry_V, ldv, K.partial, kpad);
+        else HEMO_LAUNCH(ctx, k_fg_mdot<false>, gm, FG_THREADS, smem, st, p.st, seg, ctx->kry_V, ldv, K.partial, kpad);
+        HEMO_LAUNCH(ctx, k_fg_mdot_final, m, 128, 0, st, p.st, gm, K.partial, p.scale, p.hcol);
     }
     HEMO_PROF_END(ctx, HEMO_PROF_MDOT);
     if (ctx->comm && (rc = hemo_comm_allreduce_j(ctx, p.hcol, m + 1))) return rc;
     HEMO_PROF_BEGIN(ctx, HEMO_PROF_MAXPY);
-    k_fg_maxpy<<<fg_grid(N, 1), FG_THREADS, sizeof(double) * 3 * (m + 2), st>>>(p.st, seg, N, ctx->kry_V, ldv, p.hcol, m, K.partial,
-                                                                               p.normsq, ctx->comm ? 0 : 1, p.H, p.cs, p.sn, p.g,
-                                                                               p.scale);
-    HEMO_LAUNCH_CHECK(ctx);
+    HEMO_LAUNCH(ctx, k_fg_maxpy, fg_grid(N, 1), FG_THREADS, sizeof(double) * 3 * (m + 2), st, p.st, seg, N, ctx->kry_V, ldv,
+                p.hcol, m, K.partial, p.normsq, ctx->comm ? 0 : 1, p.H, p.cs, p.sn, p.g, p.scale);
     HEMO_PROF_END(ctx, HEMO_PROF_MAXPY);
     if (ctx->comm) {
         if ((rc = hemo_comm_allreduce_j(ctx, p.normsq, 1))) return rc;
-        k_fg_givens<<<1, 64, sizeof(double) * 3 * (m + 2), st>>>(p.st, m, p.hcol, p.normsq, p.H, p.cs, p.sn, p.g, p.scale);
-        HEMO_LAUNCH_CHECK(ctx);
+        HEMO_LAUNCH(ctx, k_fg_givens, 1, 64, sizeof(double) * 3 * (m + 2), st, p.st, m, p.hcol, p.normsq, p.H, p.cs, p.sn, p.g,
+                    p.scale);
     }
     return 0;
+}
+
+static void fg_graph_stats(cudaGraph_t g, int64_t* kernels, int64_t* prog) {
+    *kernels = *prog = 0;
+    size_t nn = 0, ne = 0;
+    if (cudaGraphGetNodes(g, nullptr, &nn) != cudaSuccess || cudaGraphGetEdges_v2(g, nullptr, nullptr, nullptr, &ne) != cudaSuccess) {
+        cudaGetLastError();
+        return;
+    }
+    std::vector<cudaGraphNode_t> nodes(nn), from(ne), to(ne);
+    std::vector<cudaGraphEdgeData> data(ne);
+    if (cudaGraphGetNodes(g, nodes.data(), &nn) != cudaSuccess ||
+        cudaGraphGetEdges_v2(g, from.data(), to.data(), data.data(), &ne) != cudaSuccess) {
+        cudaGetLastError();
+        return;
+    }
+    for (cudaGraphNode_t v : nodes) {
+        cudaGraphNodeType t;
+        if (cudaGraphNodeGetType(v, &t) == cudaSuccess && t == cudaGraphNodeTypeKernel) ++*kernels;
+    }
+    for (const cudaGraphEdgeData& d : data)
+        if (d.type == cudaGraphDependencyTypeProgrammatic) ++*prog;
 }
 
 static int fg_iteration(hemo_ctx* ctx, const double* vals_dev) {
@@ -514,6 +554,7 @@
         ctx->use_graph = 0;
         return fg_iteration_body(ctx, vals_dev);
     }
+    fg_graph_stats(g, &K.iter_kernel_nodes, &K.iter_prog_edges);
     bool updated = false;
     if (K.iter_exec) {
         cudaGraphExecUpdateResultInfo info;
@@ -529,6 +570,14 @@
     K.iter_vals = vals_dev;
     HEMO_CHECK_CUDA(ctx, cudaGraphLaunch(K.iter_exec, st));
     ctx->launches += K.iter_nodes;
+    return 0;
+}
+
+extern "C" int hemo_krylov_graph_info(hemo_ctx* ctx, int64_t* kernel_nodes, int64_t* programmatic_edges) {
+    if (!ctx || !kernel_nodes || !programmatic_edges) return HEMO_EINVAL;
+    if (!ctx->kry.iter_valid) HEMO_FAIL(ctx, HEMO_ESTATE, "no FGMRES iteration graph has been captured");
+    *kernel_nodes = ctx->kry.iter_kernel_nodes;
+    *programmatic_edges = ctx->kry.iter_prog_edges;
     return 0;
 }
 
diff --git a/cfd_hemodynamic_b200/csrc/linalg.cu b/cfd_hemodynamic_b200/csrc/linalg.cu
--- a/cfd_hemodynamic_b200/csrc/linalg.cu
+++ b/cfd_hemodynamic_b200/csrc/linalg.cu
@@ -176,6 +176,8 @@
     const int lane = gt & 3;
     const bool ok = i < n;
     const int r0 = ok ? rowptr[i] : 0, r1 = ok ? rowptr[i + 1] : 0;
+    hemo_pdl_wait();
+    hemo_pdl_trigger();
     double a0 = 0.0, a1 = 0.0;
     for (int t = r0 + lane; t < r1; t += 12) {
         const int t1 = t + 4, t2 = t + 8;
@@ -223,9 +225,8 @@
 int hemo_bsr_spmv_ex(hemo_ctx* ctx, int bs, int n, const int32_t* rowptr, const int32_t* col, const areal* val,
                      const areal* x, double alpha, const areal* b, areal* y) {
     const int grid = hemo_grid((int64_t)n * 4, 256);
-    if (bs == 1) k_bsr_spmv<1><<<grid, 256, 0, ctx->stream>>>(n, rowptr, col, val, x, alpha, b, y);
-    else k_bsr_spmv<2><<<grid, 256, 0, ctx->stream>>>(n, rowptr, col, val, x, alpha, b, y);
-    HEMO_LAUNCH_CHECK(ctx);
+    if (bs == 1) HEMO_LAUNCH(ctx, k_bsr_spmv<1>, grid, 256, 0, ctx->stream, n, rowptr, col, val, x, alpha, b, y);
+    else HEMO_LAUNCH(ctx, k_bsr_spmv<2>, grid, 256, 0, ctx->stream, n, rowptr, col, val, x, alpha, b, y);
     return 0;
 }
 
@@ -459,6 +460,8 @@
 k_sub_mean_partials(int64_t n, int nparts, const double* __restrict__ partial, double* __restrict__ x) {
     __shared__ double sh[32];
     __shared__ double mean;
+    hemo_pdl_wait();
+    hemo_pdl_trigger();
     double acc = 0.0;
     for (int t = threadIdx.x; t < nparts; t += blockDim.x) acc += partial[t];
     acc = block_sum(acc, sh);
@@ -472,6 +475,8 @@
 __global__ void __launch_bounds__(RED_THREADS)
 k_sum_partial(int64_t n, const double* src, double* dst, double* __restrict__ partial) {
     __shared__ double sh[32];
+    hemo_pdl_wait();
+    hemo_pdl_trigger();
     double acc = 0.0;
     for (int64_t i = blockIdx.x * (int64_t)blockDim.x + threadIdx.x; i < n; i += (int64_t)gridDim.x * blockDim.x) {
         const double v = src[i];
@@ -486,10 +491,8 @@
     int rc = hemo_ensure_reduce(ctx, (size_t)RED_BLOCKS * 2, 512);
     if (rc) return rc;
     const int g = grid_for(n);
-    k_sum_partial<<<g, RED_THREADS, 0, ctx->stream>>>(n, src, x, ctx->red_partial);
-    HEMO_LAUNCH_CHECK(ctx);
-    k_sub_mean_partials<<<g, RED_THREADS, 0, ctx->stream>>>(n, g, ctx->red_partial, x);
-    HEMO_LAUNCH_CHECK(ctx);
+    HEMO_LAUNCH(ctx, k_sum_partial, g, RED_THREADS, 0, ctx->stream, n, src, x, ctx->red_partial);
+    HEMO_LAUNCH(ctx, k_sub_mean_partials, g, RED_THREADS, 0, ctx->stream, n, g, ctx->red_partial, x);
     return 0;
 }
 
diff --git a/cfd_hemodynamic_b200/csrc/solver.cu b/cfd_hemodynamic_b200/csrc/solver.cu
--- a/cfd_hemodynamic_b200/csrc/solver.cu
+++ b/cfd_hemodynamic_b200/csrc/solver.cu
@@ -1,4 +1,5 @@
 #include <math.h>
+#include <stdlib.h>
 
 #include "hemo_internal.cuh"
 
@@ -73,7 +74,10 @@
 
 __global__ void k_mask_nodes(int n, int bs, const uint8_t* __restrict__ mask, double* __restrict__ x) {
     const int i = blockIdx.x * blockDim.x + threadIdx.x;
-    if (i >= n || !mask[i]) return;
+    const bool masked = i < n && mask[i];
+    hemo_pdl_wait();
+    hemo_pdl_trigger();
+    if (!masked) return;
     for (int k = 0; k < bs; ++k) x[(int64_t)i * bs + k] = 0.0;
 }
 
@@ -85,10 +89,16 @@
     const int i = gt >> 2, lane = gt & 3;
     const bool ok = i < n;
     const int r0 = ok ? nrowptr[i] : 0, r1 = ok ? nrowptr[i + 1] : 0;
+    areal2 g;
+    g.x = g.y = 0;
+    int c = 0;
+    if (r0 + lane < r1) { g = a01[r0 + lane]; c = ncol[r0 + lane]; }
+    hemo_pdl_wait();
+    hemo_pdl_trigger();
     double a0 = 0.0, a1 = 0.0;
     for (int s = r0 + lane; s < r1; s += 4) {
-        const areal2 g = a01[s];
-        const double z = zp[ncol[s]];
+        if (s != r0 + lane) { g = a01[s]; c = ncol[s]; }
+        const double z = zp[c];
         a0 = fma((double)g.x, z, a0);
         a1 = fma((double)g.y, z, a1);
     }
@@ -108,19 +118,27 @@
                    const areal2* __restrict__ a01, const double* __restrict__ zp, const double* __restrict__ ru,
                    double* __restrict__ tu) {
     const int i = blockIdx.x * blockDim.x + threadIdx.x;
-    if (i >= n) return;
-    const int r0 = nrowptr[i], r1 = nrowptr[i + 1];
-    double a0 = 0.0, a1 = 0.0;
-    for (int s = r0; s < r1; s += 4) {
-        int t[4], j[4];
-        areal2 g[4];
-        double z[4];
+    const bool ok = i < n;
+    const int r0 = ok ? nrowptr[i] : 0, r1 = ok ? nrowptr[i + 1] : 0;
+    int j[4];
+    areal2 g[4];
+    auto fetch = [&](int s) {
+        int t[4];
 #pragma unroll
         for (int u = 0; u < 4; ++u) t[u] = s + u < r1 ? s + u : r1 - 1;
 #pragma unroll
         for (int u = 0; u < 4; ++u) j[u] = ncol[t[u]];
 #pragma unroll
         for (int u = 0; u < 4; ++u) g[u] = a01[t[u]];
+    };
+    if (r0 < r1) fetch(r0);
+    hemo_pdl_wait();
+    hemo_pdl_trigger();
+    if (!ok) return;
+    double a0 = 0.0, a1 = 0.0;
+    for (int s = r0; s < r1; s += 4) {
+        double z[4];
+        if (s != r0) fetch(s);
         __syncwarp(__activemask());
 #pragma unroll
         for (int u = 0; u < 4; ++u) z[u] = zp[j[u]];
@@ -143,6 +161,8 @@
     const int i = gt >> 2, lane = gt & 3;
     const bool ok = i < n;
     const int r0 = ok ? nrowptr[i] : 0, r1 = ok ? nrowptr[i + 1] : 0;
+    hemo_pdl_wait();
+    hemo_pdl_trigger();
     double a = 0.0;
     for (int s = r0 + lane; s < r1; s += 4) a = fma((double)val[s], q[ncol[s]], a);
     a += __shfl_down_sync(0xffffffffu, a, 2, 4);
@@ -155,6 +175,8 @@
                                 const double* __restrict__ conv, const uint8_t* __restrict__ dofflag ,
                                 const double* __restrict__ rp, double* __restrict__ zp) {
     const int i = blockIdx.x * blockDim.x + threadIdx.x;
+    hemo_pdl_wait();
+    hemo_pdl_trigger();
     if (i >= n) return;
     double v = cm * tp[i] / mass[i] + cl * qp[i];
     if (conv) v += cc * conv[i] / mass[i];
@@ -235,9 +257,11 @@
         if ((rc = hemo_comm_allreduce_j(ctx, ctx->coarse_rhs, nc))) break;
         cudaStream_t saved = cc->stream;
         const bool saved_cap = cc->capturing;
+        const int saved_pdl = cc->pdl;
         const int64_t before = cc->launches;
         cc->stream = side;
         cc->capturing = ctx->capturing;
+        cc->pdl = ctx->pdl;
         cc->opts.cheb_degree = ctx->opts.cheb_degree;
         cc->opts.cheb_degree_pre = ctx->opts.cheb_degree_pre;
         cc->opts.cheb_ratio = ctx->opts.cheb_ratio;
@@ -245,6 +269,7 @@
         ctx->launches += cc->launches - before;
         cc->stream = saved;
         cc->capturing = saved_cap;
+        cc->pdl = saved_pdl;
         if (rc) ctx->err = cc->err;
     } while (0);
     ctx->stream = main_st;
@@ -459,10 +484,7 @@
         if ((rc = hemo_copy_remove_mean(ctx, n, rp, tp))) return rc;
     } else {
         HEMO_CHECK_CUDA(ctx, cudaMemcpyAsync(tp, rp, sizeof(double) * n, cudaMemcpyDeviceToDevice, st));
-        if (ctx->pc_mask) {
-            k_mask_nodes<<<hemo_grid(n, 256), 256, 0, st>>>(n, 1, ctx->pc_mask, tp);
-            HEMO_LAUNCH_CHECK(ctx);
-        }
+        if (ctx->pc_mask) HEMO_LAUNCH(ctx, k_mask_nodes, hemo_grid(n, 256), 256, 0, st, n, 1, ctx->pc_mask, tp);
         if (ctx->opts.project_pressure && (rc = hemo_remove_mean(ctx, n, tp))) return rc;
     }
     if (ctx->coarse_ctx && (rc = coarse_pressure_fork(ctx, tp))) return rc;
@@ -474,27 +496,21 @@
     }
     const bool pcd = ctx->npconv_coef != 0.0 && ctx->npconv;
     if (pcd) {
-        k_node_spmv_scalar<<<hemo_grid((int64_t)n * 4, 256), 256, 0, st>>>(n, ctx->nrowptr, ctx->ncol, ctx->npconv, qp,
-                                                                          ctx->pc_tmp_u2);
-        HEMO_LAUNCH_CHECK(ctx);
-    }
-    k_schur_combine<<<hemo_grid(n, 256), 256, 0, st>>>(n, ctx->opts.schur_mass_coef, ctx->opts.schur_lap_coef,
-                                                       ctx->npconv_coef, tp, ctx->mass, qp,
-                                                       pcd ? ctx->pc_tmp_u2 : nullptr, pressure_flags(ctx), rp, zp);
-    HEMO_LAUNCH_CHECK(ctx);
+        HEMO_LAUNCH(ctx, k_node_spmv_scalar, hemo_grid((int64_t)n * 4, 256), 256, 0, st, n, ctx->nrowptr, ctx->ncol, ctx->npconv,
+                    qp, ctx->pc_tmp_u2);
+    }
+    HEMO_LAUNCH(ctx, k_schur_combine, hemo_grid(n, 256), 256, 0, st, n, ctx->opts.schur_mass_coef, ctx->opts.schur_lap_coef,
+                ctx->npconv_coef, tp, ctx->mass, qp, pcd ? ctx->pc_tmp_u2 : nullptr, pressure_flags(ctx), rp, zp);
     if (ctx->opts.project_pressure && (rc = hemo_remove_mean(ctx, n, zp))) return rc;
     }
     if (ctx->dim == 3)
         return hemo_tet_velocity_solve(ctx, vals_dev, ru, zp, tu, ctx->pc_tmp_u2, zu, 4 * ctx->opts.amg_cycles_u, 2.0 / 3.0);
     if (n >= 32768 && ctx->nnz_node <= 12 * (int64_t)n)
-        k_a01_residual_row<<<hemo_grid(n, 256), 256, 0, st>>>(n, ctx->nrowptr, ctx->ncol, ctx->a01, zp, ru, tu);
+        HEMO_LAUNCH(ctx, k_a01_residual_row, hemo_grid(n, 256), 256, 0, st, n, ctx->nrowptr, ctx->ncol, ctx->a01, zp, ru, tu);
     else
-        k_a01_residual<<<hemo_grid((int64_t)n * 4, 256), 256, 0, st>>>(n, ctx->nrowptr, ctx->ncol, ctx->a01, zp, ru, tu);
-    HEMO_LAUNCH_CHECK(ctx);
-    if (ctx->pc_mask) {
-        k_mask_nodes<<<hemo_grid(n, 256), 256, 0, st>>>(n, 2, ctx->pc_mask, tu);
-        HEMO_LAUNCH_CHECK(ctx);
-    }
+        HEMO_LAUNCH(ctx, k_a01_residual, hemo_grid((int64_t)n * 4, 256), 256, 0, st, n, ctx->nrowptr, ctx->ncol, ctx->a01, zp, ru,
+                    tu);
+    if (ctx->pc_mask) HEMO_LAUNCH(ctx, k_mask_nodes, hemo_grid(n, 256), 256, 0, st, n, 2, ctx->pc_mask, tu);
     if ((rc = hemo_amg_vcycle(ctx, &ctx->amg[0], tu, zu, ctx->opts.amg_cycles_u))) return rc;
     return 0;
 }
@@ -582,6 +598,8 @@
     ctx->opts.schur_lap_coef = 1.0;
     ctx->opts.cheb_ratio = 4.0;
     ctx->opts.cheb_degree_pre = 0;
+    const char* pdl = getenv("HEMO_PDL");
+    ctx->pdl = pdl && atoi(pdl) == 0 ? 0 : 1;
     *out = ctx;
     return 0;
 }
diff --git a/include/hemo.h b/include/hemo.h
--- a/include/hemo.h
+++ b/include/hemo.h
@@ -152,6 +152,7 @@
 int hemo_pc_apply(hemo_ctx* ctx, const double* vals_dev, const double* r_dev, double* z_dev);
 int hemo_fgmres(hemo_ctx* ctx, const double* vals_dev, const double* b_dev, double* y_dev,
                 int* its_out, double* rel_resid_out);
+int hemo_krylov_graph_info(hemo_ctx* ctx, int64_t* kernel_nodes, int64_t* programmatic_edges);
 
 #ifdef __cplusplus
 }
```

Result: faster. 50.35 million, median of 6 (+8.3%).
